# flybirdtian/pytorch_distributed_mnist

Measured on AMD Instinct MI355X. Metric: images/sec (whole node) MNIST CNN DDP at 1/2/4/8 MI355X, higher is better.
Workload: dtype bf16; 1 GPU; model=mnist_cnn, global_batch=256, batch_per_rank=256, parallelism=dp1, optimizer=sgd, graphs=True, grad_transport=local, epoch_steps=235, tail_batch_per_rank=96, conv2_products=bf16 MFMA, fp32 accumulation

## Files before the change

csrc/bind.cpp:

```cpp
#include <c10/core/DeviceGuard.h>
#include <c10/hip/HIPStream.h>
#include <torch/extension.h>

#include "kernels.h"
#include "xgmi.h"

namespace py = pybind11;

void xgmi_fill_exchange(py::handle reducer, int bucket, XgmiExch& x);
void register_comm(py::module& m);
void register_xgmi(py::module& m);

namespace {

hipStream_t cur_stream(const at::Tensor& t) {
  return c10::hip::getCurrentHIPStream(t.get_device()).stream();
}

void need(const at::Tensor& t, at::ScalarType dt, const char* name) {
  TORCH_CHECK(t.is_cuda(), name, " must be a HIP device tensor");
  TORCH_CHECK(t.scalar_type() == dt, name, " has dtype ", t.scalar_type(), ", expected ", dt);
  TORCH_CHECK(t.is_contiguous(), name, " must be contiguous");
}

void need_numel(const at::Tensor& t, int64_t n, const char* name) {
  TORCH_CHECK(t.numel() >= n, name, " has ", t.numel(), " elements, need >= ", n);
}

void need_aligned(const void* p, int bytes, const char* name) {
  TORCH_CHECK(reinterpret_cast<uintptr_t>(p) % bytes == 0, name, " must be ", bytes,
              "-byte aligned");
}

template <typename T>
T* ptr(const at::Tensor& t) { return reinterpret_cast<T*>(t.data_ptr()); }

unsigned* opt_sync(const c10::optional<at::Tensor>& t) {
  if (!t.has_value() || !t->defined()) return nullptr;
  TORCH_CHECK(t->is_cuda() && t->scalar_type() == at::kInt && t->is_contiguous() &&
                  t->numel() >= XG_LOC_WORDS, "xgmi sync words must be an int32 device tensor of ",
              XG_LOC_WORDS);
  return reinterpret_cast<unsigned*>(t->data_ptr());
}

unsigned* xg_step(const c10::optional<at::Tensor>& t) {
  unsigned* p = opt_sync(t);
  return p ? p + XG_LOC_STEP : nullptr;
}

int64_t* opt_i64(const c10::optional<at::Tensor>& t) {
  if (!t.has_value() || !t->defined()) return nullptr;
  need(*t, at::kLong, "counter");
  return ptr<int64_t>(*t);
}

LrSched opt_lr_sched(const c10::optional<py::tuple>& t, const int64_t* c1) {
  LrSched ls;
  if (!t.has_value()) return ls;
  TORCH_CHECK(t->size() == 3, "lr_sched: (table, cursor, lr)");
  TORCH_CHECK(c1 != nullptr, "lr_sched: the learning rate moves on with the optimizer-step "
                             "counter, which this launch does not advance (c1 is None)");
  const at::Tensor table = (*t)[0].cast<at::Tensor>();
  const at::Tensor cursor = (*t)[1].cast<at::Tensor>();
  const at::Tensor lr = (*t)[2].cast<at::Tensor>();
  need(table, at::kDouble, "lr_sched table");
  need(cursor, at::kLong, "lr_sched cursor");
  need(lr, at::kDouble, "lr_sched lr");
  TORCH_CHECK(table.numel() >= 1 && table.numel() <= INT32_MAX, "lr_sched table: 1..2^31-1 entries");
  TORCH_CHECK(cursor.numel() == 1 && lr.numel() == 1, "lr_sched cursor / lr: one element each");
  ls.table = table.data_ptr<double>();
  ls.n = (int)table.numel();
  ls.cursor = cursor.data_ptr<int64_t>();
  ls.lr = lr.data_ptr<double>();
  return ls;
}

float check_smoothing(double e) {
  TORCH_CHECK(e >= 0.0 && e <= 1.0, "label_smoothing must be in 0..1, got ", e);
  return (float)e;
}

void check_data(const at::Tensor& images, const at::Tensor& labels, const at::Tensor& idx,
                const at::Tensor& ctr, int64_t bfull, int64_t B) {
  need(images, at::kByte, "images");
  need(labels, at::kInt, "labels");
  need(idx, at::kInt, "idx");
  need(ctr, at::kLong, "ctr");
  TORCH_CHECK(images.dim() == 2 && images.size(1) == 784, "images must be [N, 784]");
  TORCH_CHECK(labels.numel() == images.size(0), "labels must be [N]");
  TORCH_CHECK(B >= 1 && B <= bfull, "batch ", B, " must be in [1, ", bfull, "]");
  TORCH_CHECK(ctr.numel() >= 1, "ctr must hold at least one counter");
  need_aligned(images.data_ptr(), 4, "images");
}

StepRows step_rows(int64_t bfull, int64_t spe, int64_t nrow) {
  if (spe > 0)
    TORCH_CHECK(nrow % 2 == 0 && (spe - 1) * bfull < nrow / 2 && spe * bfull >= nrow / 2,
                "epoch geometry: ", spe, " steps of ", bfull, " rows do not cover an epoch of ",
                nrow / 2, " rows");
  return StepRows{(int)bfull, (int)spe};
}

void lin_train(at::Tensor images, at::Tensor labels, c10::optional<at::Tensor> idx, at::Tensor ctr,
               int64_t bfull, int64_t B, at::Tensor W, at::Tensor b, at::Tensor slab,
               c10::optional<at::Tensor> metrics, c10::optional<at::Tensor> c1, int64_t spe,
               c10::optional<py::tuple> lr_sched, double label_smoothing) {
  c10::DeviceGuard g(images.device());
  const float eps = check_smoothing(label_smoothing);
  const bool gather = idx.has_value() && idx->defined();
  TORCH_CHECK(!(gather && spe > 0), "an epoch geometry needs the epoch buffer (idx None)");
  int64_t nrow;
  if (gather) {
    check_data(images, labels, *idx, ctr, bfull, B);
    nrow = idx->numel();
  } else {
    need(images, at::kByte, "images");
    need(labels, at::kInt, "labels");
    need(ctr, at::kLong, "ctr");
    TORCH_CHECK(images.dim() == 2 && images.size(1) == 784 && images.size(0) >= B,
                "images must be [>=B, 784]");
    TORCH_CHECK(labels.numel() == images.size(0), "labels must be [N]");
    TORCH_CHECK(B >= 1 && B <= bfull, "batch ", B, " must be in [1, ", bfull, "]");
    nrow = images.size(0);
  }
  need_aligned(images.data_ptr(), 16, "images");
  need(W, at::kFloat, "W");
  need(b, at::kFloat, "b");
  need(slab, at::kFloat, "slab");
  TORCH_CHECK(W.numel() == LIN_N * LIN_K && b.numel() == LIN_N, "W/b must be [10,784]/[10]");
  need_aligned(W.data_ptr(), 16, "W");
  const int64_t nblk = (B + LIN_ROWS - 1) / LIN_ROWS;
  need_numel(slab, nblk * LIN_SLAB, "slab");
  need_aligned(slab.data_ptr(), 16, "slab");
  double* mp = nullptr;
  if (metrics.has_value() && metrics->defined()) {
    need(*metrics, at::kDouble, "metrics");
    need_numel(*metrics, 3, "metrics");
    mp = metrics->data_ptr<double>();
  }
  launch_lin_train(images.data_ptr<uint8_t>(), labels.data_ptr<int32_t>(),
                   gather ? idx->data_ptr<int32_t>() : nullptr, nrow, ctr.data_ptr<int64_t>(),
                   step_rows(bfull, spe, nrow), (int)B, W.data_ptr<float>(), b.data_ptr<float>(),
                   slab.data_ptr<float>(), mp, opt_i64(c1), cur_stream(images),
                   opt_lr_sched(lr_sched, opt_i64(c1)), eps);
}

void lin_reduce(at::Tensor slab, int64_t B, at::Tensor gW, at::Tensor gb,
                c10::optional<at::Tensor> c0, c10::optional<at::Tensor> xg,
                c10::optional<at::Tensor> metrics) {
  c10::DeviceGuard g(slab.device());
  need(slab, at::kFloat, "slab");
  need(gW, at::kFloat, "gW");
  need(gb, at::kFloat, "gb");
  const int64_t nblk = (B + LIN_ROWS - 1) / LIN_ROWS;
  need_numel(slab, nblk * LIN_SLAB, "slab");
  TORCH_CHECK(gW.numel() == LIN_N * LIN_K && gb.numel() == LIN_N, "bad grad views");
  double* mp = nullptr;
  if (metrics.has_value() && metrics->defined()) {
    need(*metrics, at::kDouble, "metrics");
    need_numel(*metrics, 3, "metrics");
    mp = metrics->data_ptr<double>();
  }
  launch_lin_reduce(slab.data_ptr<float>(), (int)nblk, gW.data_ptr<float>(), gb.data_ptr<float>(),
                    opt_i64(c0), xg_step(xg), mp, cur_stream(slab));
}

void lin_eval(at::Tensor images, at::Tensor labels, at::Tensor W, at::Tensor b,
              at::Tensor metrics) {
  c10::DeviceGuard g(images.device());
  need(images, at::kByte, "images");
  need(labels, at::kInt, "labels");
  need(W, at::kFloat, "W");
  need(b, at::kFloat, "b");
  need(metrics, at::kDouble, "metrics");
  TORCH_CHECK(images.dim() == 2 && images.size(1) == 784, "images must be [N, 784]");
  TORCH_CHECK(labels.numel() == images.size(0), "labels must be [N]");
  TORCH_CHECK(W.numel() == LIN_N * LIN_K && b.numel() == LIN_N, "W/b must be [10,784]/[10]");
  need_numel(metrics, 3, "metrics");
  need_aligned(images.data_ptr(), 16, "images");
  need_aligned(W.data_ptr(), 16, "W");
  if (images.size(0) == 0) return;
  launch_lin_eval(images.data_ptr<uint8_t>(), labels.data_ptr<int32_t>(), (int)images.size(0),
                  W.data_ptr<float>(), b.data_ptr<float>(), metrics.data_ptr<double>(),
                  cur_stream(images));
}

void gather_epoch(at::Tensor images, at::Tensor labels, at::Tensor idx, at::Tensor out_images,
                  at::Tensor out_labels, c10::optional<at::Tensor> ctr, c10::optional<at::Tensor> step,
                  int64_t step_value, int64_t max_wgs) {
  c10::DeviceGuard g(images.device());
  need(images, at::kByte, "images");
  need(labels, at::kInt, "labels");
  need(out_images, at::kByte, "out_images");
  need(out_labels, at::kInt, "out_labels");
  TORCH_CHECK(idx.scalar_type() == at::kInt && idx.is_contiguous(), "idx must be contiguous int32");
  const int32_t* ip = nullptr;
  if (idx.is_cuda()) {
    ip = idx.data_ptr<int32_t>();
  } else {
    TORCH_CHECK(idx.is_pinned(), "a host idx must be pinned (device-mapped) memory");
    void* dp = nullptr;
    const hipError_t e = hipHostGetDevicePointer(&dp, idx.data_ptr(), 0);
    TORCH_CHECK(e == hipSuccess && dp != nullptr, "hipHostGetDevicePointer: ", hipGetErrorString(e));
    ip = static_cast<const int32_t*>(dp);
  }
  TORCH_CHECK(images.dim() == 2 && images.size(1) == 784, "images must be [N, 784]");
  const int64_t n = idx.numel();
  TORCH_CHECK(out_images.numel() >= n * 784 && out_labels.numel() >= n, "output too small");
  need_aligned(images.data_ptr(), 16, "images");
  need_aligned(out_images.data_ptr(), 16, "out_images");
  int64_t* cp = nullptr;
  int nctr = 0;
  if (ctr.has_value() && ctr->defined()) {
    need(*ctr, at::kLong, "ctr");
    TORCH_CHECK(ctr->numel() <= 256, "ctr: at most 256 counters");
    cp = ptr<int64_t>(*ctr);
    nctr = (int)ctr->numel();
  }
  int64_t* sp = nullptr;
  if (step.has_value() && step->defined()) {
    need(*step, at::kLong, "step");
    sp = ptr<int64_t>(*step);
  }
  launch_gather_epoch(images.data_ptr<uint8_t>(), labels.data_ptr<int32_t>(), ip, (int)n,
                      (int)images.size(0), out_images.data_ptr<uint8_t>(),
                      out_labels.data_ptr<int32_t>(), cp, nctr, sp, step_value, (int)max_wgs,
                      cur_stream(images));
}

void gather_epoch_augment(at::Tensor images, at::Tensor labels, at::Tensor idx,
                          at::Tensor out_images, at::Tensor out_labels,
                          c10::optional<at::Tensor> ctr, c10::optional<at::Tensor> step,
                          int64_t step_value, int64_t max_wgs, at::Tensor cosq, at::Tensor sinq,
                          at::Tensor invz, int64_t shift, int64_t epoch, uint64_t seed) {
  c10::DeviceGuard g(images.device());
  need(images, at::kByte, "images");
  need(labels, at::kInt, "labels");
  need(out_images, at::kByte, "out_images");
  need(out_labels, at::kInt, "out_labels");
  need(cosq, at::kInt, "cosq");
  need(sinq, at::kInt, "sinq");
  need(invz, at::kInt, "invz");
  need_numel(cosq, 1024, "cosq");
  need_numel(sinq, 1024, "sinq");
  need_numel(invz, 64, "invz");
  TORCH_CHECK(shift >= 0 && shift <= 8, "shift must be in 0..8, got ", shift);
  TORCH_CHECK(epoch >= 0 && epoch <= 0xffffffffLL, "epoch must fit 32 bits, got ", epoch);
  TORCH_CHECK(idx.scalar_type() == at::kInt && idx.is_contiguous(), "idx must be contiguous int32");
  const int32_t* ip = nullptr;
  if (idx.is_cuda()) {
    ip = idx.data_ptr<int32_t>();
  } else {
    TORCH_CHECK(idx.is_pinned(), "a host idx must be pinned (device-mapped) memory");
    void* dp = nullptr;
    const hipError_t e = hipHostGetDevicePointer(&dp, idx.data_ptr(), 0);
    TORCH_CHECK(e == hipSuccess && dp != nullptr, "hipHostGetDevicePointer: ", hipGetErrorString(e));
    ip = static_cast<const int32_t*>(dp);
  }
  TORCH_CHECK(images.dim() == 2 && images.size(1) == 784, "images must be [N, 784]");
  TORCH_CHECK(images.size(0) >= 1 && labels.numel() == images.size(0), "labels must be [N >= 1]");
  const int64_t n = idx.numel();
  TORCH_CHECK(out_images.numel() >= n * 784 && out_labels.numel() >= n, "output too small");
  need_aligned(images.data_ptr(), 16, "images");
  need_aligned(out_images.data_ptr(), 16, "out_images");
  int64_t* cp = nullptr;
  int nctr = 0;
  if (ctr.has_value() && ctr->defined()) {
    need(*ctr, at::kLong, "ctr");
    TORCH_CHECK(ctr->numel() <= 256, "ctr: at most 256 counters");
    cp = ptr<int64_t>(*ctr);
    nctr = (int)ctr->numel();
  }
  int64_t* sp = nullptr;
  if (step.has_value() && step->defined()) {
    need(*step, at::kLong, "step");
    sp = ptr<int64_t>(*step);
  }
  launch_gather_epoch_augment(images.data_ptr<uint8_t>(), labels.data_ptr<int32_t>(), ip, (int)n,
                              (int)images.size(0), out_images.data_ptr<uint8_t>(),
                              out_labels.data_ptr<int32_t>(), cp, nctr, sp, step_value,
                              (int)max_wgs, cosq.data_ptr<int32_t>(), sinq.data_ptr<int32_t>(),
                              invz.data_ptr<int32_t>(), (int)shift, (uint32_t)epoch, seed,
                              cur_stream(images));
}

void optim_step(int64_t kind, at::Tensor p, at::Tensor g, at::Tensor m, c10::optional<at::Tensor> v,
                at::Tensor lr, at::Tensor step, double beta1, double beta2, double eps, double wd,
                double momentum, double dampening, bool nesterov, double grad_scale,
                std::vector<py::tuple> segs, c10::optional<at::Tensor> xg, int64_t signal_ch,
                std::vector<int64_t> waits, double timeout_s, c10::optional<at::Tensor> bump,
                c10::optional<py::tuple> metrics, py::object xchg, int64_t xchg_bucket) {
  c10::DeviceGuard dg(p.device());
  need(p, at::kFloat, "params");
  need(g, at::kFloat, "grads");
  need(m, at::kFloat, "state m");
  need(lr, at::kDouble, "lr");
  need(step, at::kLong, "step");
  TORCH_CHECK(g.numel() == p.numel() && m.numel() == p.numel(), "arena size mismatch");
  TORCH_CHECK(kind == OPT_ADAM || kind == OPT_SGD, "bad optimizer kind");
  OptArgs a{};
  a.p = p.data_ptr<float>();
  a.g = g.data_ptr<float>();
  a.m = m.data_ptr<float>();
  a.v = nullptr;
  if (kind == OPT_ADAM) {
    TORCH_CHECK(v.has_value() && v->defined(), "adam needs exp_avg_sq");
    need(*v, at::kFloat, "state v");
    TORCH_CHECK(v->numel() == p.numel(), "arena size mismatch");
    a.v = v->data_ptr<float>();
  }
  a.lr = lr.data_ptr<double>();
  a.step = step.data_ptr<int64_t>();
  a.beta1_d = beta1;
  a.beta2_d = beta2;
  a.beta1 = (float)beta1;
  a.beta2 = (float)beta2;
  a.eps = (float)eps;
  a.wd = (float)wd;
  a.momentum = (float)momentum;
  a.dampening = (float)dampening;
  a.nesterov = nesterov ? 1 : 0;
  a.grad_scale = (float)grad_scale;
  TORCH_CHECK(!segs.empty() && segs.size() <= OPT_MAX_SEG, "1..8 optimizer segments");
  a.nseg = (int)segs.size();
  for (size_t i = 0; i < segs.size(); ++i) {
    const auto& t = segs[i];
    OptSeg& s = a.seg[i];
    s.offset = t[0].cast<int64_t>();
    s.rows = (int32_t)t[1].cast<int64_t>();
    s.cols = (int32_t)t[2].cast<int64_t>();
    TORCH_CHECK(s.offset >= 0 && s.rows >= 1 && s.cols >= 1 &&
                    s.offset + (int64_t)s.rows * s.cols <= p.numel(), "segment out of range");
    TORCH_CHECK(s.offset % 4 == 0, "segment offsets must be 16-byte aligned");
    s.shadow = nullptr;
    s.shadow_t = nullptr;
    s.shadow_lo = nullptr;
    s.slab = nullptr;
    s.nslab = 0;
    s.slab_col0 = 0;
    s.slab_stride = 0;
    s.wait_ch = -1;
    s.wait_mult = 0;
    if (!waits.empty()) {
      TORCH_CHECK(waits.size() == 2 * segs.size(), "waits must hold (channel, mult) per segment");
      s.wait_ch = (int32_t)waits[2 * i];
      s.wait_mult = (uint32_t)waits[2 * i + 1];
      TORCH_CHECK(s.wait_ch >= -1 && s.wait_ch < XG_MAX_CH, "bad wait channel");
    }
    if (t.size() > 5 && !t[5].is_none()) {
      auto sl = t[5].cast<py::tuple>();
      auto st = sl[0].cast<at::Tensor>();
      need(st, at::kFloat, "gradient slab");
      s.nslab = (int32_t)sl[1].cast<int64_t>();
      s.slab_col0 = (int32_t)sl[2].cast<int64_t>();
      s.slab_stride = sl[3].cast<int64_t>();
      const int64_t numel = (int64_t)s.rows * s.cols;
      TORCH_CHECK(s.nslab >= 1 && numel >= 4 && s.slab_col0 % 4 == 0 && s.slab_stride % 4 == 0 &&
                      s.slab_col0 + ((numel + 3) / 4) * 4 <= s.slab_stride &&
                      st.numel() >= (int64_t)s.nslab * s.slab_stride, "gradient slab geometry");
      need_aligned(st.data_ptr(), 16, "gradient slab");
      s.slab = st.data_ptr<float>();
    }
    if (!t[3].is_none()) {
      auto sh = t[3].cast<at::Tensor>();
      need(sh, at::kBFloat16, "shadow");
      TORCH_CHECK(sh.numel() == (int64_t)s.rows * s.cols, "shadow size mismatch");
      need_aligned(sh.data_ptr(), 8, "shadow");
      s.shadow = ptr<__bf16>(sh);
    }
    if (!t[4].is_none()) {
      auto sh = t[4].cast<at::Tensor>();
      need(sh, at::kBFloat16, "shadow_t");
      TORCH_CHECK(sh.numel() == (int64_t)s.rows * s.cols, "shadow_t size mismatch");
      s.shadow_t = ptr<__bf16>(sh);
    }
    if (t.size() > 9 && !t[9].is_none()) {
      auto sh = t[9].cast<at::Tensor>();
      need(sh, at::kBFloat16, "shadow_lo");
      TORCH_CHECK(sh.numel() == (int64_t)s.rows * s.cols, "shadow_lo size mismatch");
      need_aligned(sh.data_ptr(), 8, "shadow_lo");
      s.shadow_lo = ptr<__bf16>(sh);
    }
    s.tonly = (t.size() > 6 && !t[6].is_none() && t[6].cast<bool>()) ? 1 : 0;
    s.tfrag = (t.size() > 7 && !t[7].is_none() && t[7].cast<bool>()) ? 1 : 0;
    s.sfrag = (t.size() > 8 && !t[8].is_none() && t[8].cast<bool>()) ? 1 : 0;
    TORCH_CHECK(s.shadow_lo == nullptr || (s.shadow != nullptr && s.shadow_t == nullptr && !s.sfrag),
                "a lo shadow goes with a row-major shadow and no transposed copy");
    if (s.sfrag)
      TORCH_CHECK(s.shadow != nullptr && s.rows % 16 == 0 && s.cols % 32 == 0,
                  "a fragment-major shadow needs a 2-D segment with rows % 16 == 0 and cols % 32 == 0 "
                  "(a row shard of it starts on a 16-row fragment boundary)");
    if (s.tfrag)
      TORCH_CHECK(s.shadow_t != nullptr && s.rows % 32 == 0 && s.cols % 16 == 0,
                  "a fragment-major shadow_t needs rows % 32 == 0 and cols % 16 == 0");
    if (s.tonly) {
      TORCH_CHECK(s.shadow != nullptr && s.shadow_t != nullptr && s.slab == nullptr,
                  "a transpose-only segment needs shadow and shadow_t and no slab");
      need_aligned(s.shadow, 16, "shadow");
    }
  }
  a.xg = opt_sync(xg);
  a.xg_signal_ch = (int)signal_ch;
  a.xg_timeout = (long long)(timeout_s * 1e8);
  a.bump = opt_i64(bump);
  a.metrics = nullptr;
  a.mslab = nullptr;
  if (metrics.has_value()) {
    const auto& mt = *metrics;
    TORCH_CHECK(mt.size() == 5, "metrics: (slab, nslab, col, stride, metrics)");
    auto st = mt[0].cast<at::Tensor>();
    auto mv = mt[4].cast<at::Tensor>();
    need(st, at::kFloat, "metrics slab");
    need(mv, at::kDouble, "metrics");
    need_numel(mv, 3, "metrics");
    a.mnslab = (int32_t)mt[1].cast<int64_t>();
    a.mcol = (int32_t)mt[2].cast<int64_t>();
    a.mstride = mt[3].cast<int64_t>();
    TORCH_CHECK(a.mnslab >= 1 && a.mcol >= 0 && a.mcol + 2 <= a.mstride &&
                    st.numel() >= (int64_t)a.mnslab * a.mstride, "metrics slab geometry");
    a.mslab = st.data_ptr<float>();
    a.metrics = mv.data_ptr<double>();
  }
  TORCH_CHECK(signal_ch >= -1 && signal_ch < XG_MAX_CH, "bad signal channel");
  TORCH_CHECK(a.xg != nullptr || (signal_ch < 0 && waits.empty()),
              "optimizer waits / signals need the xgmi sync words");
  a.xx_on = 0;
  if (!xchg.is_none()) {
    xgmi_fill_exchange(xchg, (int)xchg_bucket, a.xx);
    a.xx_on = 1;
    int64_t blk = 0;
    bool plain_seen = false;
    for (int i = 0; i < a.nseg; ++i) {
      const OptSeg& sg = a.seg[i];
      if (sg.slab == nullptr) {
        plain_seen = true;
        continue;
      }
      TORCH_CHECK(!plain_seen, "exchange: slab segments must come first");
      TORCH_CHECK(sg.offset >= a.xx.off && sg.offset + (int64_t)sg.rows * sg.cols <= a.xx.off + a.xx.n,
                  "exchange: a slab segment outside the exchanged bucket");
      TORCH_CHECK(sg.wait_ch < 0, "exchange: slab segments wait for no channel");
      blk += ((int64_t)sg.rows * sg.cols + 63) / 64;
    }
    TORCH_CHECK(blk <= XG_XSLOTS, "exchange: ", blk, " slab workgroups exceed ", XG_XSLOTS, " slots");
  }
  launch_optim((int)kind, a, cur_stream(p));
}

void ema_update(at::Tensor params, at::Tensor ema, int64_t n, double w, bool warmup, double decay,
                at::Tensor step_word, int64_t offset, bool nt) {
  need(params, at::kFloat, "params");
  need(ema, at::kFloat, "ema");
  need(step_word, at::kLong, "step_word");
  c10::DeviceGuard g(params.device());
  TORCH_CHECK(ema.device() == params.device() && step_word.device() == params.device(),
              "params, ema and step_word must be on one device");
  TORCH_CHECK(n >= 1 && n <= params.numel() && n <= ema.numel(), "ema_update: n = ", n,
              " must be in 1..min(params, ema) = ", std::min(params.numel(), ema.numel()));
  TORCH_CHECK(step_word.numel() == 1, "step_word: one element");
  need_aligned(params.data_ptr(), 16, "params");
  need_aligned(ema.data_ptr(), 16, "ema");
  const char* pb = static_cast<const char*>(params.data_ptr());
  const char* eb = static_cast<const char*>(ema.data_ptr());
  TORCH_CHECK(pb + 4 * n <= eb || eb + 4 * n <= pb, "params and ema overlap");
  TORCH_CHECK(decay > 0.0 && decay < 1.0, "ema decay must be in (0, 1), got ", decay);
  TORCH_CHECK(w >= 0.0 && w <= 1.0 && (double)(float)w == w,
              "ema weight must be a float32 value in 0..1, got ", w);
  EmaArgs a;
  a.p = ptr<const float>(params);
  a.e = ptr<float>(ema);
  a.n = n;
  a.w = (float)w;
  a.warmup = warmup ? 1 : 0;
  a.decay = decay;
  a.step = ptr<const int64_t>(step_word);
  a.offset = offset;
  launch_ema_update(a, nt, cur_stream(params));
}

void xgmi_wait(at::Tensor sync, int64_t signal_ch, std::vector<int64_t> waits, double timeout_s) {
  c10::DeviceGuard g(sync.device());
  unsigned* loc = opt_sync(sync);
  TORCH_CHECK(waits.size() % 2 == 0 && waits.size() <= 8, "waits: up to 4 (channel, mult) pairs");
  TORCH_CHECK(signal_ch >= -1 && signal_ch < XG_MAX_CH, "bad signal channel");
  int ch[4];
  unsigned mult[4];
  const int n = (int)waits.size() / 2;
  for (int i = 0; i < n; ++i) {
    TORCH_CHECK(waits[2 * i] >= 0 && waits[2 * i] < XG_MAX_CH, "bad wait channel");
    ch[i] = (int)waits[2 * i];
    mult[i] = (unsigned)waits[2 * i + 1];
  }
  launch_xgmi_wait(loc, (int)signal_ch, n, ch, mult, (long long)(timeout_s * 1e8),
                   cur_stream(sync));
}

void debug_spin(double seconds) {
  TORCH_CHECK(seconds > 0 && seconds <= 30, "debug_spin: 0 < seconds <= 30");
  launch_debug_spin((long long)(seconds * 1e8), c10::hip::getCurrentHIPStream().stream());
}

void need_min(const at::Tensor& t, at::ScalarType dt, int64_t n, const char* name) {
  need(t, dt, name);
  need_numel(t, n, name);
  need_aligned(t.data_ptr(), 16, name);
}

static FcUpdate make_fc_update(const c10::optional<py::tuple>& t);

void cnn_fwd(at::Tensor images, at::Tensor labels, c10::optional<at::Tensor> idx,
             c10::optional<at::Tensor> ctr, int64_t bfull, int64_t B, at::Tensor w1, at::Tensor b1,
             at::Tensor w2, at::Tensor b2, at::Tensor pool, at::Tensor pmask,
             c10::optional<at::Tensor> xg, at::Tensor ylab, int64_t bands,
             c10::optional<at::Tensor> a1g, c10::optional<at::Tensor> xng, int64_t spe,
             c10::optional<py::tuple> fc_carry, c10::optional<py::tuple> fc_carry_wait) {
  c10::DeviceGuard g(images.device());
  FcUpdate fcc = make_fc_update(fc_carry);
  if (fc_carry_wait.has_value()) {
    const py::tuple& w = *fc_carry_wait;
    TORCH_CHECK(fcc.kind >= 0 && w.size() == 4, "fc_carry_wait: (sync, channel, mult, timeout_s) "
                "with fc_carry");
    fcc.wloc = opt_sync(w[0].cast<at::Tensor>());
    fcc.wch = (int)w[1].cast<int64_t>();
    fcc.wmult = (unsigned)w[2].cast<int64_t>();
    fcc.wtimeout = (long long)(w[3].cast<double>() * 1e8);
    TORCH_CHECK(fcc.wloc != nullptr && fcc.wch >= 0 && fcc.wch < XG_MAX_CH && fcc.wmult >= 1,
                "fc_carry_wait: bad channel / multiplier");
  }
  if (fcc.kind >= 0) {
    TORCH_CHECK(fcc.shadow_t_next != nullptr, "fc_carry: the W1^T copy (entry 16) is required");
    const bool training = (xg.has_value() && xg->defined()) || (a1g.has_value() && a1g->defined());
    TORCH_CHECK(training, "fc_carry: training launches only");
  }
  const FcUpdate* pfcc = fcc.kind >= 0 ? &fcc : nullptr;
  TORCH_CHECK(bands == 1 || bands == 2 || bands == 3 || bands == 6, "bands must be 1, 2, 3 or 6");
  const bool gather = idx.has_value() && idx->defined();
  const bool counted = ctr.has_value() && ctr->defined();
  if (gather) {
    TORCH_CHECK(counted, "ctr required with idx");
    check_data(images, labels, *idx, *ctr, bfull, B);
  } else if (counted) {
    need(images, at::kByte, "images");
    need(labels, at::kInt, "labels");
    need(*ctr, at::kLong, "ctr");
    TORCH_CHECK(images.dim() == 2 && images.size(1) == 784 && images.size(0) >= B, "images");
    TORCH_CHECK(B >= 1 && B <= bfull, "batch must be in [1, bfull]");
    need_aligned(images.data_ptr(), 4, "images");
  } else {
    need(images, at::kByte, "images");
    need(labels, at::kInt, "labels");
    TORCH_CHECK(images.dim() == 2 && images.size(1) == 784 && images.size(0) >= B,
                "images must be [>=B, 784]");
    need_aligned(images.data_ptr(), 4, "images");
  }
  TORCH_CHECK(B >= 1, "B must be >= 1");
  need(w1, at::kFloat, "w1");
  need(b1, at::kFloat, "b1");
  need(b2, at::kFloat, "b2");
  TORCH_CHECK(w1.numel() == 32 * 9 && b1.numel() == 32 && b2.numel() == 64, "conv1/conv2 bias");
  need_aligned(w1.data_ptr(), 16, "w1");
  need_aligned(b1.data_ptr(), 16, "b1");
  need_aligned(b2.data_ptr(), 16, "b2");
  need_min(w2, at::kBFloat16, 64 * 288, "w2");
  need_min(pool, at::kBFloat16, B * CNN_FEAT, "pool");
  need_min(pmask, at::kByte, B * CNN_FEAT, "pmask");
  need(ylab, at::kInt, "ylab");
  need_numel(ylab, B, "ylab");
  const bool train = xg.has_value() && xg->defined();
  if (train) need_min(*xg, at::kByte, B * 784, "xg");
  const int32_t* pidx = gather ? idx->data_ptr<int32_t>() : nullptr;
  const int64_t nrow = gather ? idx->numel() : images.size(0);
  const int64_t* pctr = counted ? ctr->data_ptr<int64_t>() : nullptr;
  uint8_t* pxg = train ? xg->data_ptr<uint8_t>() : nullptr;
  if (bands > 1) {
    __bf16* pa1 = nullptr;
    __bf16* pxn = nullptr;
    if (a1g.has_value() && a1g->defined()) {
      TORCH_CHECK(xng.has_value() && xng->defined(), "a1g needs xng");
      need_min(*a1g, at::kBFloat16, B * 676 * 32, "a1g");
      need_min(*xng, at::kBFloat16, B * 784, "xng");
      need_aligned(a1g->data_ptr(), 16, "a1g");
      need_aligned(xng->data_ptr(), 16, "xng");
      pa1 = ptr<__bf16>(*a1g);
      pxn = ptr<__bf16>(*xng);
    }
    launch_cnn_fwd_band(images.data_ptr<uint8_t>(), labels.data_ptr<int32_t>(), pidx, nrow, pctr,
                        step_rows(bfull, pidx ? 0 : spe, nrow), (int)B, (int)bands, w1.data_ptr<float>(), b1.data_ptr<float>(),
                        ptr<__bf16>(w2), b2.data_ptr<float>(), ptr<__bf16>(pool),
                        pmask.data_ptr<uint8_t>(), pa1, pxn, pxg, ylab.data_ptr<int32_t>(),
                        pfcc, cur_stream(images));
  } else {
    launch_cnn_fwd(images.data_ptr<uint8_t>(), labels.data_ptr<int32_t>(), pidx, nrow, pctr,
                   step_rows(bfull, pidx ? 0 : spe, nrow), (int)B, w1.data_ptr<float>(), b1.data_ptr<float>(), ptr<__bf16>(w2),
                   b2.data_ptr<float>(), ptr<__bf16>(pool), pmask.data_ptr<uint8_t>(), pxg,
                   ylab.data_ptr<int32_t>(), pfcc, cur_stream(images));
  }
}

void fc1_fwd(at::Tensor pool, at::Tensor wf1, at::Tensor part, int64_t B, int64_t splitk) {
  c10::DeviceGuard g(pool.device());
  TORCH_CHECK(B >= 1, "B must be >= 1");
  TORCH_CHECK(splitk >= 1 && (32 % splitk == 0 || 96 % splitk == 0),
              "splitk must divide 32 or 96");
  need_min(pool, at::kBFloat16, B * CNN_FEAT, "pool");
  need_min(wf1, at::kBFloat16, (int64_t)CNN_HID * CNN_FEAT, "wf1");
  need_min(part, at::kFloat, splitk * B * CNN_HID, "part");
  launch_fc1_fwd(ptr<__bf16>(pool), ptr<__bf16>(wf1), part.data_ptr<float>(), (int)B, (int)splitk,
                 cur_stream(pool));
}

struct HeadOut {
  __bf16 *dh = nullptr, *dht = nullptr;
  float *slab = nullptr, *dh32 = nullptr;
};

HeadOut check_head(const at::Tensor& part, int64_t splitk, int64_t B, const at::Tensor& bf1,
                   const at::Tensor& wf2, const at::Tensor& bf2, const at::Tensor& ylab, bool train,
                   const c10::optional<at::Tensor>& dh, const c10::optional<at::Tensor>& dht,
                   int64_t ldt, const c10::optional<at::Tensor>& slab, const at::Tensor& metrics,
                   const c10::optional<at::Tensor>& dh32) {
  TORCH_CHECK(B >= 1, "B must be >= 1");
  need_min(part, at::kFloat, splitk * B * CNN_HID, "part");
  need_min(bf1, at::kFloat, CNN_HID, "bf1");
  need_min(wf2, at::kFloat, CNN_NCLS * CNN_HID, "wf2");
  need(bf2, at::kFloat, "bf2");
  TORCH_CHECK(bf2.numel() == CNN_NCLS, "bf2");
  need(ylab, at::kInt, "ylab");
  need_numel(ylab, B, "ylab");
  need(metrics, at::kDouble, "metrics");
  need_numel(metrics, 3, "metrics");
  HeadOut o;
  if (train) {
    TORCH_CHECK(ldt % 32 == 0 && ldt >= B, "ldt must be a multiple of 32 and >= B");
    TORCH_CHECK(slab, "train mode needs slab");
    if (dh32.has_value() && dh32->defined()) {
      need_min(*dh32, at::kFloat, ldt * CNN_HID, "dh32");
      need_aligned(dh32->data_ptr(), 8, "dh32");
      o.dh32 = dh32->data_ptr<float>();
    } else {
      TORCH_CHECK(dh && dht, "train mode needs dh and dht (or dh32)");
      need_min(*dh, at::kBFloat16, ldt * CNN_HID, "dh");
      need_min(*dht, at::kBFloat16, ldt * CNN_HID, "dht");
      o.dh = ptr<__bf16>(*dh);
      o.dht = ptr<__bf16>(*dht);
    }
    need_min(*slab, at::kFloat, (int64_t)cnn_head_blocks((int)(ldt / CNN_HEAD_ROWS)) * CNN_HEAD_SLAB,
             "head slab");
    o.slab = slab->data_ptr<float>();
  }
  return o;
}

void cnn_head(at::Tensor part, int64_t splitk, int64_t B, at::Tensor bf1, at::Tensor wf2,
              at::Tensor bf2, at::Tensor ylab, bool train, c10::optional<at::Tensor> dh,
              c10::optional<at::Tensor> dht, int64_t ldt, c10::optional<at::Tensor> slab,
              at::Tensor metrics, c10::optional<at::Tensor> c0, c10::optional<at::Tensor> c1,
              c10::optional<at::Tensor> xg, c10::optional<at::Tensor> dh32,
              c10::optional<py::tuple> lr_sched) {
  c10::DeviceGuard g(part.device());
  TORCH_CHECK(train || !lr_sched.has_value(), "lr_sched: only a training head advances it");
  const HeadOut o = check_head(part, splitk, B, bf1, wf2, bf2, ylab, train, dh, dht, ldt, slab,
                               metrics, dh32);
  launch_cnn_head(part.data_ptr<float>(), (int)splitk, (int)B, bf1.data_ptr<float>(),
                  wf2.data_ptr<float>(), bf2.data_ptr<float>(), ylab.data_ptr<int32_t>(), train, o.dh,
                  o.dht, (int)ldt, o.slab, metrics.data_ptr<double>(), opt_i64(c0), opt_i64(c1),
                  train ? xg_step(xg) : nullptr, o.dh32, cur_stream(part),
                  opt_lr_sched(lr_sched, opt_i64(c1)));
}

void cnn_head_smooth(at::Tensor part, int64_t splitk, int64_t B, at::Tensor bf1, at::Tensor wf2,
                     at::Tensor bf2, at::Tensor ylab, c10::optional<at::Tensor> dh,
                     c10::optional<at::Tensor> dht, int64_t ldt, c10::optional<at::Tensor> slab,
                     at::Tensor metrics, c10::optional<at::Tensor> c0, c10::optional<at::Tensor> c1,
                     c10::optional<at::Tensor> xg, c10::optional<at::Tensor> dh32,
                     double label_smoothing, c10::optional<py::tuple> lr_sched) {
  c10::DeviceGuard g(part.device());
  const HeadOut o = check_head(part, splitk, B, bf1, wf2, bf2, ylab, true, dh, dht, ldt, slab,
                               metrics, dh32);
  const float eps = check_smoothing(label_smoothing);
  launch_cnn_head_smooth(part.data_ptr<float>(), (int)splitk, (int)B, bf1.data_ptr<float>(),
                         wf2.data_ptr<float>(), bf2.data_ptr<float>(), ylab.data_ptr<int32_t>(),
                         o.dh, o.dht, (int)ldt, o.slab, opt_i64(c0), opt_i64(c1), xg_step(xg),
                         o.dh32, eps, cur_stream(part), opt_lr_sched(lr_sched, opt_i64(c1)));
}

const uint32_t* check_dropout(const at::Tensor& epoch, int64_t T) {
  need(epoch, at::kInt, "epoch");
  need_numel(epoch, 1, "epoch");
  TORCH_CHECK(T >= 0 && T <= (int64_t)DROPOUT_MAX_T, "T must be in 0..", DROPOUT_MAX_T, ", got ", T);
  return reinterpret_cast<const uint32_t*>(epoch.data_ptr<int32_t>());
}

void cnn_head_dropout(at::Tensor part, int64_t splitk, int64_t B, at::Tensor bf1, at::Tensor wf2,
                      at::Tensor bf2, at::Tensor ylab, c10::optional<at::Tensor> dh,
                      c10::optional<at::Tensor> dht, int64_t ldt, c10::optional<at::Tensor> slab,
                      at::Tensor metrics, c10::optional<at::Tensor> c0,
                      c10::optional<at::Tensor> c1, c10::optional<at::Tensor> xg,
                      c10::optional<at::Tensor> dh32, at::Tensor epoch, uint64_t seed, int64_t T,
                      double scale, c10::optional<py::tuple> lr_sched, double label_smoothing) {
  c10::DeviceGuard g(part.device());
  const HeadOut o = check_head(part, splitk, B, bf1, wf2, bf2, ylab, true, dh, dht, ldt, slab,
                               metrics, dh32);
  const uint32_t* pe = check_dropout(epoch, T);
  TORCH_CHECK(scale >= 1.0 && scale <= 65536.0 / (65536.0 - DROPOUT_MAX_T) + 1e-6,
              "scale must be 65536 / (65536 - T), got ", scale);
  const float eps = check_smoothing(label_smoothing);
  launch_cnn_head_dropout(part.data_ptr<float>(), (int)splitk, (int)B, bf1.data_ptr<float>(),
                          wf2.data_ptr<float>(), bf2.data_ptr<float>(), ylab.data_ptr<int32_t>(),
                          o.dh, o.dht, (int)ldt, o.slab, opt_i64(c0), opt_i64(c1), xg_step(xg),
                          o.dh32, pe, seed, (uint32_t)T, (float)scale, cur_stream(part),
                          opt_lr_sched(lr_sched, opt_i64(c1)), eps);
}

at::Tensor dropout_mask_rows(at::Tensor ylab, at::Tensor epoch, uint64_t seed, int64_t T) {
  c10::DeviceGuard g(ylab.device());
  need(ylab, at::kInt, "ylab");
  TORCH_CHECK(ylab.dim() == 1 && ylab.numel() >= 1, "ylab must be [B >= 1]");
  const uint32_t* pe = check_dropout(epoch, T);
  const int64_t B = ylab.numel();
  at::Tensor out = at::empty({B, (int64_t)CNN_HID}, ylab.options().dtype(at::kByte));
  launch_dropout_mask_rows(ylab.data_ptr<int32_t>(), (int)B, pe, seed, (uint32_t)T,
                           out.data_ptr<uint8_t>(), cur_stream(ylab));
  return out;
}

struct PredictOut {
  float* logp;
  int32_t* pred;
  int64_t* confusion;
  double* metrics;
};
PredictOut check_predict_out(int64_t B, bool labelled, const at::Tensor& logp, const at::Tensor& pred,
                             const c10::optional<at::Tensor>& confusion,
                             const c10::optional<at::Tensor>& metrics) {
  PredictOut o{};
  need(logp, at::kFloat, "logp");
  need_numel(logp, B * CNN_NCLS, "logp");
  need(pred, at::kInt, "pred");
  need_numel(pred, B, "pred");
  o.logp = logp.data_ptr<float>();
  o.pred = pred.data_ptr<int32_t>();
  if (confusion.has_value() && confusion->defined()) {
    TORCH_CHECK(labelled, "confusion needs labels");
    need(*confusion, at::kLong, "confusion");
    TORCH_CHECK(confusion->numel() == CNN_NCLS * CNN_NCLS, "confusion must be [10, 10]");
    o.confusion = confusion->data_ptr<int64_t>();
  }
  if (metrics.has_value() && metrics->defined()) {
    TORCH_CHECK(labelled, "metrics need labels");
    need(*metrics, at::kDouble, "metrics");
    need_numel(*metrics, 3, "metrics");
    o.metrics = metrics->data_ptr<double>();
  }
  return o;
}

void cnn_predict_head(at::Tensor part, int64_t splitk, int64_t B, at::Tensor bf1, at::Tensor wf2,
                      at::Tensor bf2, c10::optional<at::Tensor> ylab, at::Tensor logp,
                      at::Tensor pred, c10::optional<at::Tensor> confusion,
                      c10::optional<at::Tensor> metrics) {
  c10::DeviceGuard g(part.device());
  TORCH_CHECK(B >= 1 && B <= INT32_MAX / (CNN_NCLS * 4), "B must be in [1, 2^31 / 40)");
  TORCH_CHECK(splitk >= 1, "splitk must be >= 1");
  need_min(part, at::kFloat, splitk * B * CNN_HID, "part");
  need_min(bf1, at::kFloat, CNN_HID, "bf1");
  need_min(wf2, at::kFloat, CNN_NCLS * CNN_HID, "wf2");
  need(bf2, at::kFloat, "bf2");
  TORCH_CHECK(bf2.numel() == CNN_NCLS, "bf2");
  const bool labelled = ylab.has_value() && ylab->defined();
  if (labelled) {
    need(*ylab, at::kInt, "ylab");
    need_numel(*ylab, B, "ylab");
  }
  const PredictOut o = check_predict_out(B, labelled, logp, pred, confusion, metrics);
  launch_cnn_predict_head(part.data_ptr<float>(), (int)splitk, (int)B, bf1.data_ptr<float>(),
                          wf2.data_ptr<float>(), bf2.data_ptr<float>(),
                          labelled ? ylab->data_ptr<int32_t>() : nullptr, o.logp, o.pred,
                          o.confusion, o.metrics, cur_stream(part));
}

void lin_predict(at::Tensor images, c10::optional<at::Tensor> labels, at::Tensor W, at::Tensor b,
                 at::Tensor logp, at::Tensor pred, c10::optional<at::Tensor> confusion,
                 c10::optional<at::Tensor> metrics) {
  c10::DeviceGuard g(images.device());
  need(images, at::kByte, "images");
  need(W, at::kFloat, "W");
  need(b, at::kFloat, "b");
  TORCH_CHECK(images.dim() == 2 && images.size(1) == 784, "images must be [N, 784]");
  const int64_t n = images.size(0);
  TORCH_CHECK(n <= INT32_MAX / LIN_K, "too many rows for one launch");
  const bool labelled = labels.has_value() && labels->defined();
  if (labelled) {
    need(*labels, at::kInt, "labels");
    TORCH_CHECK(labels->numel() == n, "labels must be [N]");
  }
  TORCH_CHECK(W.numel() == LIN_N * LIN_K && b.numel() == LIN_N, "W/b must be [10,784]/[10]");
  need_aligned(images.data_ptr(), 16, "images");
  need_aligned(W.data_ptr(), 16, "W");
  const PredictOut o = check_predict_out(n, labelled, logp, pred, confusion, metrics);
  if (n == 0) return;
  launch_lin_predict(images.data_ptr<uint8_t>(), labelled ? labels->data_ptr<int32_t>() : nullptr,
                     (int)n, W.data_ptr<float>(), b.data_ptr<float>(), o.logp, o.pred, o.confusion,
                     o.metrics, cur_stream(images));
}


static FcUpdate make_fc_update(const c10::optional<py::tuple>& t) {
  FcUpdate u{};
  u.kind = -1;
  if (!t.has_value()) return u;
  const py::tuple& a = *t;
  TORCH_CHECK(a.size() >= 16 && a.size() <= 18, "fc_update: 16 to 18 entries");
  u.kind = (int)a[0].cast<int64_t>();
  TORCH_CHECK(u.kind == OPT_SGD, "fc_update: SGD-momentum only (Adam runs in the optimizer kernel)");
  auto p = a[1].cast<at::Tensor>(), g = a[2].cast<at::Tensor>(), m = a[3].cast<at::Tensor>();
  auto sh = a[5].cast<at::Tensor>(), lr = a[6].cast<at::Tensor>(), st = a[7].cast<at::Tensor>();
  need(p, at::kFloat, "fc p");
  need(g, at::kFloat, "fc g");
  need(m, at::kFloat, "fc m");
  need(sh, at::kBFloat16, "fc shadow");
  need(lr, at::kDouble, "lr");
  need(st, at::kLong, "step");
  u.numel = p.numel();
  TORCH_CHECK(u.numel == (int64_t)CNN_HID * CNN_FEAT && g.numel() == u.numel &&
                  m.numel() == u.numel && sh.numel() == u.numel, "fc_update: fc1 weight sizes");
  for (const void* q : {p.data_ptr(), g.data_ptr(), m.data_ptr()}) need_aligned(q, 16, "fc_update fp32");
  need_aligned(sh.data_ptr(), 16, "fc_update shadow");
  u.p = p.data_ptr<float>();
  u.g = g.data_ptr<float>();
  u.m = m.data_ptr<float>();
  u.v = nullptr;
  u.shadow = ptr<__bf16>(sh);
  u.lr = lr.data_ptr<double>();
  u.step = st.data_ptr<int64_t>();
  u.beta1_d = a[8].cast<double>();
  u.beta2_d = a[9].cast<double>();
  u.beta1 = (float)u.beta1_d;
  u.beta2 = (float)u.beta2_d;
  u.eps = (float)a[10].cast<double>();
  u.wd = (float)a[11].cast<double>();
  u.momentum = (float)a[12].cast<double>();
  u.dampening = (float)a[13].cast<double>();
  u.nesterov = a[14].cast<bool>() ? 1 : 0;
  u.grad_scale = (float)a[15].cast<double>();
  u.shadow_t_next = nullptr;
  u.store_grad = (a.size() == 18 && !a[17].is_none()) ? (a[17].cast<bool>() ? 1 : 0) : 1;
  if (a.size() >= 17 && !a[16].is_none()) {
    auto t2 = a[16].cast<at::Tensor>();
    need(t2, at::kBFloat16, "fc shadow_t_next");
    TORCH_CHECK(t2.numel() == u.numel, "fc_update: shadow_t_next is one W1^T copy");
    need_aligned(t2.data_ptr(), 16, "fc_update shadow_t_next");
    u.shadow_t_next = ptr<__bf16>(t2);
  }
  return u;
}

void fc1_bwd(at::Tensor dh, at::Tensor dht, int64_t ldt, at::Tensor pool, at::Tensor wf1t,
             int64_t B, at::Tensor gwf1, at::Tensor dpool, at::Tensor head_slab, at::Tensor gwf2,
             at::Tensor gbf2, at::Tensor gbf1, at::Tensor metrics,
             c10::optional<py::tuple> fc_update) {
  c10::DeviceGuard g(dh.device());
  TORCH_CHECK(B >= 1 && ldt % 32 == 0 && ldt >= B, "bad ldt/B");
  need_min(dh, at::kBFloat16, ldt * CNN_HID, "dh");
  need_min(dht, at::kBFloat16, ldt * CNN_HID, "dht");
  need_min(pool, at::kBFloat16, B * CNN_FEAT, "pool");
  need_min(wf1t, at::kBFloat16, (int64_t)CNN_FEAT * CNN_HID, "wf1t");
  need_min(dpool, at::kBFloat16, B * CNN_FEAT, "dpool");
  need(gwf1, at::kFloat, "gwf1");
  need(gwf2, at::kFloat, "gwf2");
  need(gbf2, at::kFloat, "gbf2");
  need(gbf1, at::kFloat, "gbf1");
  TORCH_CHECK(gwf1.numel() == (int64_t)CNN_HID * CNN_FEAT && gwf2.numel() == CNN_NCLS * CNN_HID &&
                  gbf2.numel() == CNN_NCLS && gbf1.numel() == CNN_HID, "fc grad views");
  const int64_t hb = cnn_head_blocks((int)(ldt / CNN_HEAD_ROWS));
  need_min(head_slab, at::kFloat, hb * CNN_HEAD_SLAB, "head slab");
  need(metrics, at::kDouble, "metrics");
  need_numel(metrics, 3, "metrics");
  const FcUpdate fcu = make_fc_update(fc_update);
  if (fcu.shadow_t_next != nullptr) {
    const char* r0 = reinterpret_cast<const char*>(wf1t.data_ptr());
    const char* w0 = reinterpret_cast<const char*>(fcu.shadow_t_next);
    const int64_t nb = (int64_t)CNN_FEAT * CNN_HID * 2;
    TORCH_CHECK(w0 + nb <= r0 || r0 + nb <= w0, "fc_update: shadow_t_next overlaps the W1^T being read");
  }
  launch_fc1_bwd(ptr<__bf16>(dh), ptr<__bf16>(dht), (int)ldt, ptr<__bf16>(pool), ptr<__bf16>(wf1t),
                 (int)B, gwf1.data_ptr<float>(), ptr<__bf16>(dpool), head_slab.data_ptr<float>(),
                 (int)hb, gwf2.data_ptr<float>(), gbf2.data_ptr<float>(), gbf1.data_ptr<float>(),
                 metrics.data_ptr<double>(), fcu, cur_stream(dh));
}

static int64_t conv_blocks(int64_t B, int64_t ipb, int64_t bands) {
  return bands > 1 ? B * bands : (int64_t)cnn_bwd_blocks((int)B, (int)ipb);
}

void cnn_bwd(at::Tensor xg, at::Tensor w1, at::Tensor b1, at::Tensor dpool, at::Tensor pmask,
             at::Tensor w2t, int64_t B, int64_t ipb, at::Tensor slab,
             c10::optional<at::Tensor> xg_sync, int64_t bands, c10::optional<at::Tensor> a1g,
             c10::optional<at::Tensor> xng) {
  c10::DeviceGuard g(xg.device());
  TORCH_CHECK(B >= 1 && ipb >= 1, "bad B/ipb");
  TORCH_CHECK(bands == 1 || ((bands == 2 || bands == 3 || bands == 6) && ipb == 1),
              "bands must be 1, or 2 / 3 / 6 with one image per band group");
  need_min(xg, at::kByte, B * 784, "xg");
  need(w1, at::kFloat, "w1");
  need(b1, at::kFloat, "b1");
  TORCH_CHECK(w1.numel() == 32 * 9 && b1.numel() == 32, "conv1 weight/bias");
  need_min(dpool, at::kBFloat16, B * CNN_FEAT, "dpool");
  need_min(pmask, at::kByte, B * CNN_FEAT, "pmask");
  need_min(w2t, at::kBFloat16, 288 * 64, "w2t");
  need_min(slab, at::kFloat, conv_blocks(B, ipb, bands) * CNN_CONV_SLAB, "conv slab");
  need_aligned(slab.data_ptr(), 16, "conv slab");
  if (bands > 1) {
    TORCH_CHECK(a1g.has_value() && xng.has_value(), "the band backward needs a1g and xng");
    need_min(*a1g, at::kBFloat16, B * 676 * 32, "a1g");
    need_min(*xng, at::kBFloat16, B * 784, "xng");
    need_aligned(a1g->data_ptr(), 16, "a1g");
    need_aligned(xng->data_ptr(), 16, "xng");
    launch_cnn_bwd_band(ptr<__bf16>(*a1g), ptr<__bf16>(*xng), ptr<__bf16>(dpool),
                        pmask.data_ptr<uint8_t>(), ptr<__bf16>(w2t), (int)B, (int)bands,
                        slab.data_ptr<float>(), opt_sync(xg_sync), cur_stream(xg));
  } else
    launch_cnn_bwd(xg.data_ptr<uint8_t>(), w1.data_ptr<float>(), b1.data_ptr<float>(),
                   ptr<__bf16>(dpool), pmask.data_ptr<uint8_t>(), ptr<__bf16>(w2t), (int)B, (int)ipb,
                   slab.data_ptr<float>(), opt_sync(xg_sync), cur_stream(xg));
}

void conv_reduce(at::Tensor slab, int64_t nblk, at::Tensor gw2, at::Tensor gb2, at::Tensor gw1,
                 at::Tensor gb1) {
  c10::DeviceGuard g(slab.device());
  need_min(slab, at::kFloat, nblk * CNN_CONV_SLAB, "conv slab");
  need_aligned(slab.data_ptr(), 16, "conv slab");
  TORCH_CHECK(nblk >= 1, "nblk must be >= 1");
  need(gw2, at::kFloat, "gw2");
  need(gb2, at::kFloat, "gb2");
  need(gw1, at::kFloat, "gw1");
  need(gb1, at::kFloat, "gb1");
  TORCH_CHECK(gw2.numel() == 64 * 288 && gb2.numel() == 64 && gw1.numel() == 288 &&
                  gb1.numel() == 32, "conv grad views");
  launch_conv_reduce(slab.data_ptr<float>(), (int)nblk, gw2.data_ptr<float>(),
                     gb2.data_ptr<float>(), gw1.data_ptr<float>(), gb1.data_ptr<float>(),
                     cur_stream(slab));
}

int64_t cnn_bwd_nblk(int64_t B, int64_t ipb, int64_t bands) { return conv_blocks(B, ipb, bands); }

static float* w2x_ptr(const c10::optional<at::Tensor>& w2x) {
  TORCH_CHECK(w2x.has_value() && w2x->defined(), "the split-bf16 path needs the w2x buffer");
  need_min(*w2x, at::kFloat, 2 * 9 * 32 * 128 / 4, "w2x");
  need_aligned(w2x->data_ptr(), 16, "w2x");
  return w2x->data_ptr<float>();
}

void f32_fwd(at::Tensor images, at::Tensor labels, c10::optional<at::Tensor> ctr, int64_t bfull,
             int64_t B, at::Tensor w1, at::Tensor b1, at::Tensor w2, at::Tensor b2,
             at::Tensor pool, c10::optional<at::Tensor> pmask, c10::optional<at::Tensor> a1g,
             c10::optional<at::Tensor> xng, at::Tensor ylab, int64_t spe, bool x3,
             c10::optional<at::Tensor> w2x, c10::optional<at::Tensor> w2s) {
  c10::DeviceGuard g(images.device());
  need(images, at::kByte, "images");
  need(labels, at::kInt, "labels");
  TORCH_CHECK(images.dim() == 2 && images.size(1) == 784 && images.size(0) >= 1, "images [N, 784]");
  TORCH_CHECK(labels.numel() == images.size(0), "labels [N]");
  need_aligned(images.data_ptr(), 4, "images");
  TORCH_CHECK(B >= 1 && (!ctr.has_value() ? images.size(0) >= B : B <= bfull), "batch size");
  if (ctr.has_value()) need(*ctr, at::kLong, "ctr");
  need(w1, at::kFloat, "w1");
  need(b1, at::kFloat, "b1");
  need(w2, at::kFloat, "w2");
  need(b2, at::kFloat, "b2");
  TORCH_CHECK(w1.numel() == 288 && b1.numel() == 32 && w2.numel() == 64 * 288 && b2.numel() == 64,
              "conv weights");
  for (const void* q : {w1.data_ptr(), b1.data_ptr(), b2.data_ptr()}) need_aligned(q, 16, "conv weight");
  need_min(pool, at::kFloat, B * CNN_FEAT, "pool");
  need(ylab, at::kInt, "ylab");
  need_min(ylab, at::kInt, B, "ylab");
  const __bf16* w2sp = nullptr;
  if (x3) {
    TORCH_CHECK(w2s.has_value() && w2s->defined(), "the split-bf16 forward needs w2s");
    need(*w2s, at::kBFloat16, "w2s");
    TORCH_CHECK(w2s->numel() == 2 * 64 * 288, "w2s: hi / lo planes of conv2's weight");
    need_aligned(w2s->data_ptr(), 16, "w2s");
    w2sp = ptr<__bf16>(*w2s);
  }
  const bool train = a1g.has_value() && a1g->defined();
  if (train) {
    TORCH_CHECK(pmask.has_value() && xng.has_value(), "training needs pmask, a1g and xng");
    need_min(*pmask, at::kByte, B * CNN_FEAT, "pmask");
    need_min(*a1g, at::kFloat, B * 676 * 32, "a1g");
    need_min(*xng, at::kFloat, B * 784, "xng");
    need_aligned(a1g->data_ptr(), 16, "a1g");
    need_aligned(xng->data_ptr(), 16, "xng");
  }
  launch_f32_fwd(images.data_ptr<uint8_t>(), labels.data_ptr<int32_t>(), images.size(0),
                 ctr.has_value() ? ctr->data_ptr<int64_t>() : nullptr,
                 step_rows(bfull, ctr.has_value() ? spe : 0, images.size(0)), (int)B,
                 w1.data_ptr<float>(), b1.data_ptr<float>(), w2.data_ptr<float>(), b2.data_ptr<float>(),
                 pool.data_ptr<float>(), train ? pmask->data_ptr<uint8_t>() : nullptr,
                 train ? a1g->data_ptr<float>() : nullptr, train ? xng->data_ptr<float>() : nullptr,
                 ylab.data_ptr<int32_t>(), x3,
                 train && x3 ? w2x_ptr(w2x) : nullptr, w2sp, cur_stream(images));
}

void f32_fc1_fwd(at::Tensor pool, at::Tensor w1, at::Tensor part, int64_t B, int64_t splitk,
                 bool x3) {
  c10::DeviceGuard g(pool.device());
  TORCH_CHECK(B >= 1 && splitk >= 1 && 288 % splitk == 0, "splitk must divide 288");
  TORCH_CHECK(!x3 || 96 % splitk == 0, "split-bf16 fc1: splitk must divide 96");
  need_min(pool, at::kFloat, B * CNN_FEAT, "pool");
  need(w1, at::kFloat, "w1");
  TORCH_CHECK(w1.numel() == (int64_t)CNN_HID * CNN_FEAT, "fc1 weight");
  need_min(part, at::kFloat, splitk * B * CNN_HID, "part");
  for (const void* q : {pool.data_ptr(), w1.data_ptr()}) need_aligned(q, 16, "fc1 operand");
  launch_f32_fc1_fwd(pool.data_ptr<float>(), w1.data_ptr<float>(), part.data_ptr<float>(), (int)B,
                     (int)splitk, x3, cur_stream(pool));
}

void f32_fc1_bwd(at::Tensor dh, int64_t ldt, at::Tensor pool, at::Tensor w1, int64_t B,
                 at::Tensor gwf1, at::Tensor dpool, at::Tensor head_slab, at::Tensor gwf2,
                 at::Tensor gbf2, at::Tensor gbf1, at::Tensor metrics, bool x3) {
  c10::DeviceGuard g(dh.device());
  TORCH_CHECK(B >= 1 && ldt % 32 == 0 && ldt >= B, "ldt must be a multiple of 32 and >= B");
  need_min(dh, at::kFloat, ldt * CNN_HID, "dh32");
  need_min(pool, at::kFloat, B * CNN_FEAT, "pool");
  need(w1, at::kFloat, "w1");
  TORCH_CHECK(w1.numel() == (int64_t)CNN_HID * CNN_FEAT, "fc1 weight");
  need(gwf1, at::kFloat, "gwf1");
  TORCH_CHECK(gwf1.numel() == (int64_t)CNN_HID * CNN_FEAT, "fc1 grad");
  need_min(dpool, at::kFloat, B * CNN_FEAT, "dpool");
  const int hb = cnn_head_blocks((int)(ldt / CNN_HEAD_ROWS));
  need_min(head_slab, at::kFloat, (int64_t)hb * CNN_HEAD_SLAB, "head slab");
  need(gwf2, at::kFloat, "gwf2");
  need(gbf2, at::kFloat, "gbf2");
  need(gbf1, at::kFloat, "gbf1");
  TORCH_CHECK(gwf2.numel() == 1280 && gbf2.numel() == 10 && gbf1.numel() == 128, "head grads");
  need(metrics, at::kDouble, "metrics");
  need_numel(metrics, 3, "metrics");
  for (const void* q : {dh.data_ptr(), pool.data_ptr(), w1.data_ptr()}) need_aligned(q, 16, "fc1 operand");
  launch_f32_fc1_bwd(dh.data_ptr<float>(), (int)ldt, pool.data_ptr<float>(), w1.data_ptr<float>(),
                     (int)B, gwf1.data_ptr<float>(), dpool.data_ptr<float>(),
                     head_slab.data_ptr<float>(), hb, gwf2.data_ptr<float>(), gbf2.data_ptr<float>(),
                     gbf1.data_ptr<float>(), metrics.data_ptr<double>(), x3, cur_stream(dh));
}

void f32_conv_bwd(at::Tensor a1g, at::Tensor xng, at::Tensor dpool, at::Tensor pmask, at::Tensor w2,
                  int64_t B, at::Tensor slab, int64_t ipb, bool x3, c10::optional<at::Tensor> w2x) {
  c10::DeviceGuard g(a1g.device());
  TORCH_CHECK(B >= 1 && ipb >= 1, "B and ipb must be >= 1");
  need_min(a1g, at::kFloat, B * 676 * 32, "a1g");
  need_min(xng, at::kFloat, B * 784, "xng");
  need_min(dpool, at::kFloat, B * CNN_FEAT, "dpool");
  need_min(pmask, at::kByte, B * CNN_FEAT, "pmask");
  need(w2, at::kFloat, "w2");
  TORCH_CHECK(w2.numel() == 64 * 288, "conv2 weight");
  need_min(slab, at::kFloat, (int64_t)f32_conv_bwd_blocks((int)B, (int)ipb, x3) * CNN_CONV_SLAB,
           "conv slab");
  launch_f32_conv_bwd(a1g.data_ptr<float>(), xng.data_ptr<float>(), dpool.data_ptr<float>(),
                      pmask.data_ptr<uint8_t>(), w2.data_ptr<float>(), (int)B, (int)ipb,
                      slab.data_ptr<float>(), x3, x3 ? w2x_ptr(w2x) : nullptr, cur_stream(a1g));
}

void graph_upload(int64_t exec, int64_t device) {
  TORCH_CHECK(exec != 0, "graph_upload: graph is not instantiated");
  c10::DeviceGuard g(c10::Device(c10::kCUDA, (c10::DeviceIndex)device));
  hipStream_t s = c10::hip::getCurrentHIPStream((c10::DeviceIndex)device).stream();
  hipError_t e = hipGraphUpload(reinterpret_cast<hipGraphExec_t>(exec), s);
  TORCH_CHECK(e == hipSuccess, "hipGraphUpload: ", hipGetErrorString(e));
}

at::Tensor read_stamps(const std::string& which) {
  at::Tensor t = at::zeros({256, 16}, at::TensorOptions().dtype(at::kLong));
  auto* p = reinterpret_cast<unsigned long long*>(t.data_ptr<int64_t>());
  if (which == "fwd") read_stamps_fwd(p);
  else if (which == "head") read_stamps_head(p);
  else if (which == "fc1_bwd") read_stamps_fc1_bwd(p);
  else if (which == "fwd_band") read_stamps_fwd_band(p);
  else if (which == "bwd_band") read_stamps_bwd_band(p);
  else if (which == "f32") read_stamps_f32(p);
  else read_stamps_bwd(p);
  return t;
}

}

PYBIND11_MODULE(_C, m) {
  m.doc() = "MI355X (gfx950) kernels + RCCL runtime for pytorch_distributed_mnist_amd";
#ifdef PDM_DEBUG_BOUNDS
  m.attr("DEBUG_BOUNDS") = true;
#else
  m.attr("DEBUG_BOUNDS") = false;
#endif
  m.attr("LIN_ROWS") = LIN_ROWS;
  m.attr("LIN_SLAB") = LIN_SLAB;
  m.attr("OPT_ADAM") = OPT_ADAM;
  m.attr("OPT_SGD") = OPT_SGD;
  m.attr("XG_LOC_ERR") = XG_LOC_ERR;
  m.attr("XG_LOC_STEP") = XG_LOC_STEP;
  m.attr("XG_LOC_READY") = XG_LOC_READY;
  m.attr("XG_LOC_DONE") = XG_LOC_DONE;
  m.def("lin_train", &lin_train, py::arg("images"), py::arg("labels"), py::arg("idx"),
        py::arg("ctr"), py::arg("bfull"), py::arg("B"), py::arg("W"), py::arg("b"), py::arg("slab"),
        py::arg("metrics") = py::none(), py::arg("c1") = py::none(), py::arg("spe") = 0,
        py::arg("lr_sched") = py::none(), py::arg("label_smoothing") = 0.0);
  m.def("lin_reduce", &lin_reduce, py::arg("slab"), py::arg("B"), py::arg("gW"), py::arg("gb"),
        py::arg("c0") = py::none(), py::arg("xg") = py::none(), py::arg("metrics") = py::none());
  m.def("lin_eval", &lin_eval);
  m.def("optim_step", &optim_step, py::arg("kind"), py::arg("p"), py::arg("g"), py::arg("m"),
        py::arg("v"), py::arg("lr"), py::arg("step"), py::arg("beta1"), py::arg("beta2"),
        py::arg("eps"), py::arg("wd"), py::arg("momentum"), py::arg("dampening"),
        py::arg("nesterov"), py::arg("grad_scale"), py::arg("segs"), py::arg("xg") = py::none(),
        py::arg("signal_ch") = -1, py::arg("waits") = std::vector<int64_t>{},
        py::arg("timeout_s") = 60.0, py::arg("bump") = py::none(),
        py::arg("metrics") = py::none(), py::arg("xchg") = py::none(), py::arg("xchg_bucket") = 1);
  m.def("ema_update", &ema_update, py::arg("params"), py::arg("ema"), py::arg("n"), py::arg("w"),
        py::arg("warmup"), py::arg("decay"), py::arg("step_word"), py::arg("offset"),
        py::arg("nt") = false);
  m.def("gather_epoch", &gather_epoch, py::arg("images"), py::arg("labels"), py::arg("idx"),
        py::arg("out_images"), py::arg("out_labels"), py::arg("ctr") = py::none(),
        py::arg("step") = py::none(), py::arg("step_value") = 0, py::arg("max_wgs") = 0);
  m.def("gather_epoch_augment", &gather_epoch_augment, py::arg("images"), py::arg("labels"),
        py::arg("idx"), py::arg("out_images"), py::arg("out_labels"), py::arg("ctr") = py::none(),
        py::arg("step") = py::none(), py::arg("step_value") = 0, py::arg("max_wgs") = 0,
        py::arg("cosq"), py::arg("sinq"), py::arg("invz"), py::arg("shift"), py::arg("epoch"),
        py::arg("seed"));
  m.def("xgmi_wait", &xgmi_wait);
  m.def("debug_spin", &debug_spin, py::arg("seconds"));
  m.attr("CNN_HEAD_ROWS") = CNN_HEAD_ROWS;
  m.def("cnn_head_nblk", [](int64_t ldt) { return cnn_head_blocks((int)(ldt / CNN_HEAD_ROWS)); });
  m.attr("CNN_HEAD_SLAB") = CNN_HEAD_SLAB;
  m.attr("CNN_CONV_SLAB") = CNN_CONV_SLAB;
  m.attr("CNN_CONV_SLAB_DB2") = CNN_CONV_SLAB_DB2;
  m.attr("CNN_CONV_SLAB_DW1") = CNN_CONV_SLAB_DW1;
  m.attr("CNN_CONV_SLAB_DB1") = CNN_CONV_SLAB_DB1;
  m.def("cnn_fwd", &cnn_fwd, py::arg("images"), py::arg("labels"), py::arg("idx"), py::arg("ctr"),
        py::arg("bfull"), py::arg("B"), py::arg("w1"), py::arg("b1"), py::arg("w2"), py::arg("b2"),
        py::arg("pool"), py::arg("pmask"), py::arg("xg"), py::arg("ylab"), py::arg("bands") = 1,
        py::arg("a1g") = py::none(), py::arg("xng") = py::none(), py::arg("spe") = 0,
        py::arg("fc_carry") = py::none(), py::arg("fc_carry_wait") = py::none());
  m.def("fc1_fwd", &fc1_fwd);
  m.attr("FC1_BIG_B") = FC1_BIG_B;
  m.def("cnn_head", &cnn_head, py::arg("part"), py::arg("splitk"), py::arg("B"), py::arg("bf1"),
        py::arg("wf2"), py::arg("bf2"), py::arg("ylab"), py::arg("train"), py::arg("dh"),
        py::arg("dht"), py::arg("ldt"), py::arg("slab"), py::arg("metrics"), py::arg("c0"),
        py::arg("c1"), py::arg("xg") = py::none(), py::arg("dh32") = py::none(),
        py::arg("lr_sched") = py::none());
  m.def("cnn_head_dropout", &cnn_head_dropout, py::arg("part"), py::arg("splitk"), py::arg("B"),
        py::arg("bf1"), py::arg("wf2"), py::arg("bf2"), py::arg("ylab"), py::arg("dh"),
        py::arg("dht"), py::arg("ldt"), py::arg("slab"), py::arg("metrics"), py::arg("c0"),
        py::arg("c1"), py::arg("xg") = py::none(), py::arg("dh32") = py::none(), py::arg("epoch"),
        py::arg("seed"), py::arg("T"), py::arg("scale"), py::arg("lr_sched") = py::none(),
        py::arg("label_smoothing") = 0.0);
  m.def("cnn_head_smooth", &cnn_head_smooth, py::arg("part"), py::arg("splitk"), py::arg("B"),
        py::arg("bf1"), py::arg("wf2"), py::arg("bf2"), py::arg("ylab"), py::arg("dh"),
        py::arg("dht"), py::arg("ldt"), py::arg("slab"), py::arg("metrics"), py::arg("c0"),
        py::arg("c1"), py::arg("xg") = py::none(), py::arg("dh32") = py::none(),
        py::arg("label_smoothing"), py::arg("lr_sched") = py::none());
  m.def("dropout_mask_rows", &dropout_mask_rows, py::arg("ylab"), py::arg("epoch"),
        py::arg("seed"), py::arg("T"));
  m.def("cnn_predict_head", &cnn_predict_head, py::arg("part"), py::arg("splitk"), py::arg("B"),
        py::arg("bf1"), py::arg("wf2"), py::arg("bf2"), py::arg("ylab"), py::arg("logp"),
        py::arg("pred"), py::arg("confusion") = py::none(), py::arg("metrics") = py::none());
  m.def("lin_predict", &lin_predict, py::arg("images"), py::arg("labels"), py::arg("W"),
        py::arg("b"), py::arg("logp"), py::arg("pred"), py::arg("confusion") = py::none(),
        py::arg("metrics") = py::none());
  m.def("fc1_bwd", &fc1_bwd, py::arg("dh"), py::arg("dht"), py::arg("ldt"), py::arg("pool"),
        py::arg("wf1t"), py::arg("B"), py::arg("gwf1"), py::arg("dpool"), py::arg("head_slab"),
        py::arg("gwf2"), py::arg("gbf2"), py::arg("gbf1"), py::arg("metrics"),
        py::arg("fc_update") = py::none());
  m.def("cnn_bwd", &cnn_bwd, py::arg("xg"), py::arg("w1"), py::arg("b1"), py::arg("dpool"),
        py::arg("pmask"), py::arg("w2t"), py::arg("B"), py::arg("ipb"), py::arg("slab"),
        py::arg("xg_sync") = py::none(), py::arg("bands") = 1, py::arg("a1g") = py::none(),
        py::arg("xng") = py::none());
  m.def("conv_reduce", &conv_reduce);
  m.def("f32_fwd", &f32_fwd, py::arg("images"), py::arg("labels"), py::arg("ctr"), py::arg("bfull"),
        py::arg("B"), py::arg("w1"), py::arg("b1"), py::arg("w2"), py::arg("b2"), py::arg("pool"),
        py::arg("pmask"), py::arg("a1g"), py::arg("xng"), py::arg("ylab"), py::arg("spe") = 0,
        py::arg("x3") = false, py::arg("w2x") = py::none(), py::arg("w2s") = py::none());
  m.def("f32_fc1_fwd", &f32_fc1_fwd, py::arg("pool"), py::arg("w1"), py::arg("part"), py::arg("B"),
        py::arg("splitk"), py::arg("x3") = false);
  m.def("f32_fc1_bwd", &f32_fc1_bwd, py::arg("dh"), py::arg("ldt"), py::arg("pool"), py::arg("w1"),
        py::arg("B"), py::arg("gwf1"), py::arg("dpool"), py::arg("head_slab"), py::arg("gwf2"),
        py::arg("gbf2"), py::arg("gbf1"), py::arg("metrics"), py::arg("x3") = false);
  m.def("f32_conv_bwd", &f32_conv_bwd, py::arg("a1g"), py::arg("xng"), py::arg("dpool"),
        py::arg("pmask"), py::arg("w2"), py::arg("B"), py::arg("slab"), py::arg("ipb") = 1,
        py::arg("x3") = false, py::arg("w2x") = py::none());
  m.def("f32_conv_bwd_nblk", [](int64_t B, int64_t ipb, bool x3) {
    return (int64_t)f32_conv_bwd_blocks((int)B, (int)ipb, x3); }, py::arg("B"), py::arg("ipb") = 1,
    py::arg("x3") = false);
  m.def("cnn_bwd_nblk", &cnn_bwd_nblk, py::arg("B"), py::arg("ipb"), py::arg("bands") = 1);
  m.def("read_stamps", &read_stamps);
  m.def("graph_upload", &graph_upload);
  register_comm(m);
  register_xgmi(m);
}
```

csrc/kernels.h:

```cpp
#pragma once
#include <hip/hip_runtime.h>
#include <stdint.h>

#include "xgmi.h"


struct StepRows {
  int bfull;
  int spe;
};
__host__ __device__ __forceinline__ int64_t step_row(const StepRows g, int64_t nrow, int64_t c,
                                                     int img) {
  if (g.spe <= 0) return c * g.bfull + img;
  const uint32_t e = (uint32_t)c / (uint32_t)g.spe;
  const int64_t s = c - (int64_t)e * g.spe;
  return (int64_t)(e & 1u) * (nrow >> 1) + s * g.bfull + img;
}

struct LrSched {
  const double* table = nullptr;
  int n = 0;
  int64_t* cursor = nullptr;
  double* lr = nullptr;
};

constexpr int LIN_K = 784;
constexpr int LIN_N = 10;
constexpr int LIN_ROWS = 4;
constexpr int LIN_SLAB = 7856;
constexpr int LIN_EVAL_ROWS = 16;

void launch_lin_train(const uint8_t* images, const int32_t* labels, const int32_t* idx,
                      int64_t nrow, const int64_t* ctr, StepRows sr, int B, const float* W, const float* b,
                      float* slab, double* metrics, int64_t* c1, hipStream_t st,
                      LrSched ls = LrSched(), float label_smoothing = 0.f);
void launch_lin_reduce(const float* slab, int nblk, float* gW, float* gb, int64_t* c0, unsigned* c2,
                       double* metrics, hipStream_t st);
void launch_lin_eval(const uint8_t* images, const int32_t* labels, int n_total, const float* W,
                     const float* b, double* metrics, hipStream_t st);

void launch_gather_epoch(const uint8_t* images, const int32_t* labels, const int32_t* idx, int n,
                         int nimg, uint8_t* out_images, int32_t* out_labels, int64_t* ctr,
                         int nctr, int64_t* step, int64_t step_value, int max_wgs, hipStream_t st);
void launch_gather_epoch_augment(const uint8_t* images, const int32_t* labels, const int32_t* idx,
                                 int n, int nimg, uint8_t* out_images, int32_t* out_labels,
                                 int64_t* ctr, int nctr, int64_t* step, int64_t step_value,
                                 int max_wgs, const int32_t* cosq, const int32_t* sinq,
                                 const int32_t* invz, int shift, uint32_t epoch, uint64_t seed,
                                 hipStream_t st);

constexpr int OPT_ADAM = 0;
constexpr int OPT_SGD = 1;
constexpr int OPT_MAX_SEG = 8;

struct OptSeg {
  int64_t offset;
  int32_t rows, cols;
  int32_t first_block;
  __bf16* shadow;
  __bf16* shadow_t;
  __bf16* shadow_lo;
  const float* slab;
  int32_t nslab, slab_col0;
  int64_t slab_stride;
  int32_t wait_ch;
  uint32_t wait_mult;
  int32_t tonly;
  int32_t tfrag;
  int32_t sfrag;
};

__host__ __device__ inline int64_t frag_pos(int64_t m, int64_t k, int32_t K) {
  return (((m >> 4) * (K >> 5) + (k >> 5)) * 64 + ((k >> 3) & 3) * 16 + (m & 15)) * 8 + (k & 7);
}
__host__ __device__ inline int64_t shadow_pos(int32_t sfrag, int32_t cols, int64_t row, int64_t col) {
  return sfrag ? frag_pos(row, col, cols) : row * cols + col;
}
__host__ __device__ inline int64_t shadow_t_pos(int32_t tfrag, int32_t rows, int64_t row, int64_t col) {
  return tfrag ? frag_pos(col, row, rows) : col * rows + row;
}

struct OptArgs {
  float* p;
  const float* g;
  float* m;
  float* v;
  const double* lr;
  const int64_t* step;
  double beta1_d, beta2_d;
  float beta1, beta2, eps, wd, momentum, dampening;
  int nesterov;
  float grad_scale;
  int nseg;
  OptSeg seg[OPT_MAX_SEG];
  unsigned* xg;
  int xg_signal_ch;
  long long xg_timeout;
  int64_t* bump;
  const float* mslab;
  int32_t mnslab, mcol;
  int64_t mstride;
  double* metrics;
  int xx_on;
  XgmiExch xx;
};

void launch_optim(int kind, OptArgs& a, hipStream_t st);

struct EmaArgs {
  const float* p;
  float* e;
  int64_t n;
  float w;
  int warmup;
  double decay;
  const int64_t* step;
  int64_t offset;
};
void launch_ema_update(const EmaArgs& a, bool nt, hipStream_t st);

constexpr int FC1_BIG_B = 2048;

struct FcUpdate {
  int kind;
  int64_t numel;
  float* p;
  const float* g;
  float* m;
  float* v;
  __bf16* shadow;
  __bf16* shadow_t_next;
  const double* lr;
  const int64_t* step;
  double beta1_d, beta2_d;
  float beta1, beta2, eps, wd, momentum, dampening;
  int nesterov;
  float grad_scale;
  int store_grad;
  unsigned* wloc;
  int wch;
  unsigned wmult;
  long long wtimeout;
};

constexpr int CNN_FEAT = 9216;
constexpr int CNN_HID = 128;
constexpr int CNN_NCLS = 10;
constexpr int CNN_HEAD_ROWS = 4;
constexpr int CNN_HEAD_MAX_BLOCKS = 256;
int cnn_head_blocks(int groups);
constexpr int CNN_HEAD_SLAB = 1420;
constexpr int CNN_CONV_SLAB = 18816;
constexpr int CNN_CONV_SLAB_DB2 = 18432;
constexpr int CNN_CONV_SLAB_DW1 = 18496;
constexpr int CNN_CONV_SLAB_DB1 = 18784;

void launch_cnn_fwd(const uint8_t* images, const int32_t* labels, const int32_t* idx,
                    int64_t nrow, const int64_t* ctr, StepRows sr, int B, const float* w1, const float* b1,
                    const __bf16* w2, const float* b2, __bf16* pool, uint8_t* pmask, uint8_t* xg,
                    int32_t* ylab, const FcUpdate* fcc, hipStream_t st);
void launch_cnn_fwd_band(const uint8_t* images, const int32_t* labels, const int32_t* idx,
                         int64_t nrow, const int64_t* ctr, StepRows sr, int B, int bands,
                         const float* w1, const float* b1, const __bf16* w2, const float* b2,
                         __bf16* pool, uint8_t* pmask, __bf16* a1g, __bf16* xng, uint8_t* xg,
                         int32_t* ylab, const FcUpdate* fcc, hipStream_t st);
void launch_fc1_fwd(const __bf16* pool, const __bf16* wf1, float* part, int B, int splitk,
                    hipStream_t st);
void launch_cnn_head(const float* part, int splitk, int B, const float* bf1, const float* wf2,
                     const float* bf2, const int32_t* ylab, bool train, __bf16* dh, __bf16* dht,
                     int ldt, float* slab, double* metrics, int64_t* c0, int64_t* c1,
                     unsigned* c2, float* dh32, hipStream_t st, LrSched ls = LrSched());
void launch_cnn_head_smooth(const float* part, int splitk, int B, const float* bf1,
                            const float* wf2, const float* bf2, const int32_t* ylab, __bf16* dh,
                            __bf16* dht, int ldt, float* slab, int64_t* c0, int64_t* c1,
                            unsigned* c2, float* dh32, float label_smoothing, hipStream_t st,
                            LrSched ls = LrSched());
void launch_cnn_head_dropout(const float* part, int splitk, int B, const float* bf1,
                             const float* wf2, const float* bf2, const int32_t* ylab, __bf16* dh,
                             __bf16* dht, int ldt, float* slab, int64_t* c0, int64_t* c1,
                             unsigned* c2, float* dh32, const uint32_t* epoch, uint64_t seed,
                             uint32_t T, float scale, hipStream_t st, LrSched ls = LrSched(),
                             float label_smoothing = 0.f);
void launch_dropout_mask_rows(const int32_t* ylab, int B, const uint32_t* epoch, uint64_t seed,
                              uint32_t T, uint8_t* out, hipStream_t st);
constexpr uint32_t DROPOUT_MAX_T = 58982;
void launch_fc1_bwd(const __bf16* dh, const __bf16* dht, int ldt, const __bf16* pool,
                    const __bf16* wf1t, int B, float* gwf1, __bf16* dpool, const float* head_slab,
                    int head_blocks, float* gwf2, float* gbf2, float* gbf1, double* metrics,
                    const FcUpdate& fcu, hipStream_t st);
void launch_cnn_bwd(const uint8_t* xg, const float* w1, const float* b1, const __bf16* dpool,
                    const uint8_t* pmask, const __bf16* w2t, int B, int imgs_per_block, float* slab,
                    unsigned* xg_sync, hipStream_t st);
int cnn_bwd_blocks(int B, int imgs_per_block);
void launch_cnn_bwd_band(const __bf16* a1g, const __bf16* xng, const __bf16* dpool,
                         const uint8_t* pmask, const __bf16* w2t, int B, int bands, float* slab,
                         unsigned* xg_sync, hipStream_t st);
void launch_conv_reduce(const float* slab, int nblk, float* gw2, float* gb2, float* gw1, float* gb1,
                        hipStream_t st);

void launch_f32_fwd(const uint8_t* images, const int32_t* labels, int64_t nrow, const int64_t* ctr,
                    StepRows sr, int B, const float* w1, const float* b1, const float* w2,
                    const float* b2, float* pool, uint8_t* pmask, float* a1g, float* xng,
                    int32_t* ylab, bool x3, float* w2x, const __bf16* w2s, hipStream_t st);
void launch_f32_fc1_fwd(const float* pool, const float* w1, float* part, int B, int splitk,
                        bool x3, hipStream_t st);
void launch_f32_fc1_bwd(const float* dh, int ldt, const float* pool, const float* w1, int B,
                        float* gwf1, float* dpool, const float* head_slab, int head_blocks,
                        float* gwf2, float* gbf2, float* gbf1, double* metrics, bool x3, hipStream_t st);
int f32_conv_bwd_blocks(int B, int per, bool x3);
void launch_f32_conv_bwd(const float* a1g, const float* xng, const float* dpool,
                         const uint8_t* pmask, const float* w2, int B, int ipb, float* slab,
                         bool x3, const float* w2x, hipStream_t st);

void launch_cnn_predict_head(const float* part, int splitk, int B, const float* bf1,
                             const float* wf2, const float* bf2, const int32_t* ylab, float* logp,
                             int32_t* pred, int64_t* confusion, double* metrics, hipStream_t st);
void launch_lin_predict(const uint8_t* images, const int32_t* labels, int n_total, const float* W,
                        const float* b, float* logp, int32_t* pred, int64_t* confusion,
                        double* metrics, hipStream_t st);

void read_stamps_fwd(unsigned long long* host);
void read_stamps_head(unsigned long long* host);
void read_stamps_fc1_bwd(unsigned long long* host);
void read_stamps_bwd(unsigned long long* host);
void read_stamps_fwd_band(unsigned long long* host);
void read_stamps_bwd_band(unsigned long long* host);
void read_stamps_f32(unsigned long long* host);
```

csrc/kernels/cnn_fwd.hip:

```cpp
#include "cnn_common.h"
#include "fc_carry.h"

namespace {

using namespace cnn;

constexpr int FWD_THREADS = 512;
constexpr int F_X3 = 0;
constexpr int F_A1 = 6400;
constexpr int F_PS = F_A1 + P1 * 64;
constexpr int F_MS = F_PS + PP * C2 * 2;
constexpr int F_LUT = F_MS + PP * C2;
constexpr int F_W = F_LUT + 512;
constexpr int F_TOTAL = F_W + 1536;
static_assert(2 * F_TOTAL <= 163840 && F_A1 % 128 == 0, "cnn_fwd LDS carve");

template <bool TRAIN, bool CARRY>
__global__ __launch_bounds__(FWD_THREADS, 2) void cnn_fwd_kernel(
    const uint8_t* __restrict__ images, const int32_t* __restrict__ labels,
    const int32_t* __restrict__ idx, int64_t nrow, const int64_t* __restrict__ ctr, const StepRows sr,
    const float* __restrict__ w1, const float* __restrict__ b1, const bf16* __restrict__ w2,
    const float* __restrict__ b2, bf16* __restrict__ pool, uint8_t* __restrict__ pmask,
    uint8_t* __restrict__ xg, int32_t* __restrict__ ylab, const FcUpdate fcc, int nconv) {
  __shared__ __attribute__((aligned(16))) char smem[F_TOTAL];
  static_assert(F_TOTAL >= FCC_LDS + 4, "carried fc1 update tiles fit the forward's LDS");
  if constexpr (CARRY) {
    if ((int)blockIdx.x >= nconv) {
      fc_carry_role(fcc, blockIdx.x - nconv, gridDim.x - nconv, smem);
      return;
    }
  }
  bf16x4* x3 = reinterpret_cast<bf16x4*>(smem + F_X3);
  char* a1s = smem + F_A1;
  bf16* ps = reinterpret_cast<bf16*>(smem + F_PS);
  uint8_t* ms = reinterpret_cast<uint8_t*>(smem + F_MS);

  const int img = blockIdx.x;
  const int tid = threadIdx.x, lane = tid & 63;
  const int wave = __builtin_amdgcn_readfirstlane(tid >> 6);
  const int g = lane >> 4, i16 = lane & 15;
  PDM_STAMP(0);
  float4 wq = make_float4(0.f, 0.f, 0.f, 0.f);
  const int wt = tid - 256;
  if (wt >= 0 && wt < 96) {
    const float4* srcw = wt < 72 ? reinterpret_cast<const float4*>(w1) + wt
                         : wt < 80 ? reinterpret_cast<const float4*>(b1) + (wt - 72)
                                   : reinterpret_cast<const float4*>(b2) + (wt - 80);
    wq = *srcw;
  }
  __builtin_amdgcn_sched_barrier(0);
  const int64_t row_u = ctr ? step_row(sr, nrow, *ctr, img) : (int64_t)img;
  PDM_CHECK(row_u < nrow, "cnn_fwd sample row past the epoch", row_u, nrow);
  const int64_t row = min(row_u, nrow - 1);
  const int64_t src = idx ? (int64_t)idx[row] : row;
  uint32_t xw = 0, xn = 0;
  if (tid < 196) {
    xw = reinterpret_cast<const uint32_t*>(images + src * 784)[tid];
    xn = reinterpret_cast<const uint32_t*>(images + src * 784)[min(tid + 1, 195)];
  }
  int lab = 0;
  if (tid == 64) {
    int vz;
    asm volatile("v_mov_b32 %0, 0" : "=v"(vz));
    lab = labels[src + vz];
  }
  if (tid == 0) PDM_STAMP_VAL(8, PDM_CLOCK());
  bf16* lut = reinterpret_cast<bf16*>(smem + F_LUT);
  if (tid >= 256) lut[tid - 256] = to_bf16(pdm_normalize(tid - 256));
  float* wl = reinterpret_cast<float*>(smem + F_W);
  if (wt >= 0 && wt < 96) reinterpret_cast<float4*>(wl)[wt] = wq;
  __builtin_amdgcn_sched_barrier(0);
  __syncthreads();

  float w1v[2][4];
#pragma unroll
  for (int j = 0; j < 4; ++j)
#pragma unroll
    for (int mt = 0; mt < 2; ++mt)
      w1v[mt][j] = wl[(mt * 16 + i16) * 9 + 3 * min(g, 2) + min(j, 2)];
  f32x4 b1v[2];
#pragma unroll
  for (int mt = 0; mt < 2; ++mt) b1v[mt] = reinterpret_cast<const f32x4*>(wl + 288)[mt * 4 + g];
  if (tid < 196) {
    const bf16 v[6] = {lut[xw & 0xff], lut[(xw >> 8) & 0xff], lut[(xw >> 16) & 0xff],
                       lut[xw >> 24], lut[xn & 0xff], lut[(xn >> 8) & 0xff]};
#pragma unroll
    for (int i = 0; i < 4; ++i) x3[4 * tid + i] = bf16x4{v[i], v[i + 1], v[i + 2], bf16{}};
    if (TRAIN) st_ho<4>(reinterpret_cast<uint32_t*>(xg + (int64_t)img * 784) + tid, xw);
    if (tid == 0) PDM_STAMP_VAL(9, PDM_CLOCK());
  }
  __syncthreads();
  PDM_STAMP(1);

  __builtin_amdgcn_sched_barrier(0);
  const int nh = wave & 1;
  float b2r[2];
#pragma unroll
  for (int j = 0; j < 2; ++j) b2r[j] = wl[320 + nh * 32 + j * 16 + i16];
  bf16x8 wb[9][2];
  auto load_wb = [&](int f) {
#pragma unroll
    for (int e = 3 * f; e < 3 * f + 3; ++e)
      wb[e >> 1][e & 1] = *reinterpret_cast<const bf16x8*>(
          w2 + ((int64_t)((nh * 2 + (e & 1)) * 9 + (e >> 1)) * 64 + lane) * 8);
  };

  bf16x4 w1f[2];
#pragma unroll
  for (int mt = 0; mt < 2; ++mt)
#pragma unroll
    for (int j = 0; j < 4; ++j) w1f[mt][j] = to_bf16(g < 3 && j < 3 ? w1v[mt][j] : 0.f);
  {
    constexpr int TPW = 6;
    const int rowg = IMG * (g < 3 ? g : 0);
    const int a1c = (conv1_pair_chunk(g) ^ (i16 & 3)) << 4;
#pragma unroll
    for (int h = 0; h < TPW; h += 3) {
    bf16x4 bx[TPW];
    int vv[TPW];
#pragma unroll
    for (int k = h; k < h + 3; ++k) {
      vv[k] = (wave + 8 * k) * 16 + i16;
      bx[k] = x3[min(vv[k], IMG * H1 - 1) + rowg];
    }
#pragma unroll
    for (int k = h; k < h + 3; ++k) {
      load_wb(k);
      const int y = vv[k] / IMG, x = vv[k] - y * IMG;
      const bool ok = y < H1 && x < H1;
      bf16x4 o[2];
#pragma unroll
      for (int mt = 0; mt < 2; ++mt) {
        f32x4 acc = __builtin_amdgcn_mfma_f32_16x16x16bf16_1k(w1f[mt], bx[k], b1v[mt], 0, 0, 0);
        o[mt] = bf16x4{to_bf16(relu1(acc[0])), to_bf16(relu1(acc[1])),
                       to_bf16(relu1(acc[2])), to_bf16(relu1(acc[3]))};
      }
      const int dst = ok ? F_A1 + (vv[k] - 2 * y) * 64 + a1c : F_PS + lane * 16;
      *reinterpret_cast<uint4*>(smem + dst) = conv1_pair(o[0], o[1]);
    }
    }
  }
  __syncthreads();
  PDM_STAMP(2);

  const int q = i16 >> 2, s = i16 & 3;
  const int lp = ((s >> 1) * H1 + 2 * q + (s & 1)) * 64;
  int aoff[9];
#pragma unroll
  for (int ky = 0; ky < 3; ++ky)
#pragma unroll
    for (int kx = 0; kx < 3; ++kx)
      aoff[ky * 3 + kx] = lp + (ky * H1 + kx) * 64 + ((g ^ ((2 * q + (s & 1) + kx) & 3)) << 4);
  const int pr = wave >> 1;
  const int tt0 = pr < 2 ? 10 * pr : 20 + 8 * (pr - 2), tt1 = tt0 + (pr < 2 ? 10 : 8);
  for (int tt = tt0; tt < tt1; ++tt) {
    const int py = tt / 3, px0 = 4 * (tt - py * 3);
    const char* tb = a1s + (2 * py * H1 + 2 * px0) * 64;
    bf16x8 a[9];
#pragma unroll
    for (int t = 0; t < 9; ++t) a[t] = *reinterpret_cast<const bf16x8*>(tb + aoff[t]);
    f32x4 acc[2];
#pragma unroll
    for (int j = 0; j < 2; ++j) acc[j] = f32x4{b2r[j], b2r[j], b2r[j], b2r[j]};
#pragma unroll
    for (int t = 0; t < 9; ++t)
#pragma unroll
      for (int j = 0; j < 2; ++j)
        acc[j] = __builtin_amdgcn_mfma_f32_16x16x32_bf16(a[t], wb[t][j], acc[j], 0, 0, 0);
    const int pp = py * HP + px0 + g;
#pragma unroll
    for (int j = 0; j < 2; ++j) {
      const int co = nh * 32 + j * 16 + i16;
      const int b0 = fbits(acc[j][0]), b1 = fbits(acc[j][1]), b2 = fbits(acc[j][2]);
      const int mb = max(max(max(b0, b1), b2), fbits(acc[j][3]));
      uint32_t oh = b2 == mb ? 4u : 8u;
      oh = b1 == mb ? 2u : oh;
      oh = b0 == mb ? 1u : oh;
      const bool pos = mb > 0;
      ps[pp * C2 + co] = to_bf16(__builtin_bit_cast(float, max(mb, 0)));
      ms[pp * C2 + co] = (uint8_t)(pos ? 0x80u | oh : 0u);
    }
  }
  PDM_STAMP(3);
  if ((threadIdx.x & 63) == 0 && wave >= 1 && wave <= 6) PDM_STAMP_VAL(9 + wave, PDM_CLOCK());
  __syncthreads();
  PDM_STAMP(4);

  uint4* pout = reinterpret_cast<uint4*>(pool + (int64_t)img * FEAT);
  for (int i = tid; i < FEAT * 2 / 16; i += FWD_THREADS) st_ho<4>(pout + i, reinterpret_cast<const uint4*>(ps)[i]);
  if (TRAIN) {
    uint4* mout = reinterpret_cast<uint4*>(pmask + (int64_t)img * FEAT);
    for (int i = tid; i < FEAT / 16; i += FWD_THREADS) st_ho<4>(mout + i, reinterpret_cast<const uint4*>(ms)[i]);
  }
  if (tid == 64) st_ho<4>(ylab + img, lab);
  PDM_STAMP(5);
}

}

void launch_cnn_fwd(const uint8_t* images, const int32_t* labels, const int32_t* idx,
                    int64_t nrow, const int64_t* ctr, StepRows sr, int B, const float* w1, const float* b1,
                    const __bf16* w2, const float* b2, __bf16* pool, uint8_t* pmask, uint8_t* xg,
                    int32_t* ylab, const FcUpdate* fcc, hipStream_t st) {
  if (fcc != nullptr) {
    cnn_fwd_kernel<true, true><<<B + FCC_WGS, FWD_THREADS, 0, st>>>(
        images, labels, idx, nrow, ctr, sr, w1, b1, w2, b2, pool, pmask, xg, ylab, *fcc, B);
    return;
  }
  const FcUpdate none{};
  if (xg != nullptr)
    cnn_fwd_kernel<true, false><<<B, FWD_THREADS, 0, st>>>(images, labels, idx, nrow, ctr, sr, w1, b1,
                                                           w2, b2, pool, pmask, xg, ylab, none, B);
  else
    cnn_fwd_kernel<false, false><<<B, FWD_THREADS, 0, st>>>(images, labels, idx, nrow, ctr, sr, w1,
                                                            b1, w2, b2, pool, pmask, xg, ylab, none, B);
}

PDM_STAMP_READER(fwd)
```

csrc/kernels/fc1_bwd.hip:

```cpp
#include "cnn_common.h"
#include "optim_common.h"

namespace {

using namespace cnn;

#ifdef PDM_STAMPS
#define FC_STAMP(row, slot)                                                         \
  do {                                                                              \
    if (threadIdx.x == 0 && (row) < 256)                                            \
      pdm_stamps[(row) * 16 + (slot)] = __builtin_amdgcn_s_memtime();              \
  } while (0)
#else
#define FC_STAMP(row, slot) do { } while (0)
#endif
#ifndef PDM_DW_MT
#define PDM_DW_MT 1
#endif
constexpr int DW_MT = PDM_DW_MT;
static_assert(DW_MT == 1 || DW_MT == 2, "dW tile: 64 or 128 hidden rows");
constexpr int DW_FT = FEAT / 64;
constexpr int DW_TILES = DW_FT * (2 / DW_MT);
constexpr int DWC = 128;
constexpr int DX_COLS = 384;
constexpr int DX_TILES = FEAT / DX_COLS;
constexpr int DX_FT = DX_COLS / 64;
constexpr int NXCD = 8;
static_assert(DX_TILES % NXCD == 0 && DW_TILES % NXCD == 0, "XCD-aware tile mapping");
constexpr int HR_BLOCKS = (HEAD_SLAB + 63) / 64;

__device__ __forceinline__ int tile_off(int row, int byte) {
  return row * 128 + (byte ^ ((((row >> 1) & 1) | (((row >> 3) & 1) << 1)) << 5));
}

__global__ __launch_bounds__(256, 2) void fc1_bwd_kernel(
    const bf16* __restrict__ dh, const bf16* __restrict__ dht, int ldt,
    const bf16* __restrict__ pool, const bf16* __restrict__ wf1t, int B, float* __restrict__ gwf1,
    bf16* __restrict__ dpool, const float* __restrict__ head_slab, int head_blocks,
    float* __restrict__ gwf2, float* __restrict__ gbf2, float* __restrict__ gbf1,
    double* __restrict__ metrics, int bid_offset, const FcUpdate fcu) {
  __shared__ __attribute__((aligned(16))) char tile[2 * DWC * 128];
  const int tid = threadIdx.x, lane = tid & 63, wave = tid >> 6;
  const int g = lane >> 4, i16 = lane & 15, q = i16 >> 2, pq = i16 & 3;
  const int nd = (ldt / 32) * DX_TILES;
  const int bid = blockIdx.x + bid_offset;

  if (bid < DW_TILES) {
    const int k0 = (bid % DW_FT) * 64, n0 = (bid / DW_FT) * 64 * DW_MT;
    FC_STAMP(bid, 8);
    f32x4 acc[DW_MT][4];
#pragma unroll
    for (int i = 0; i < DW_MT; ++i)
#pragma unroll
      for (int j = 0; j < 4; ++j) acc[i][j] = f32x4{0.f, 0.f, 0.f, 0.f};
    const int srow = tid >> 3, sch = tid & 7;
    uint4 pv[DWC / 32];
    bf16x8 a[DW_MT][DWC / 32];
    auto load_chunk = [&](int c0) __attribute__((always_inline)) {
#pragma unroll
      for (int j = 0; j < DWC / 32; ++j) {
        const int row = c0 + srow + 32 * j;
        const uint4 v = *reinterpret_cast<const uint4*>(pool + (int64_t)min(row, B - 1) * FEAT +
                                                        k0 + sch * 8);
        pv[j] = row < B ? v : make_uint4(0, 0, 0, 0);
      }
#pragma unroll
      for (int mt = 0; mt < DW_MT; ++mt)
#pragma unroll
        for (int kk = 0; kk < DWC / 32; ++kk)
          a[mt][kk] = *reinterpret_cast<const bf16x8*>(
              dht + ((int64_t)((n0 / 16 + wave * DW_MT + mt) * (ldt / 32) +
                               (min(c0 + 32 * kk, ldt - 32) >> 5)) * 64 + lane) * 8);
    };
    load_chunk(0);
    float fpv[DW_MT][4][4], fmv[DW_MT][4][4];
    double fc_lr = 0.0;
    int64_t fc_t = 0;
    if (fcu.kind >= 0) {
      fc_lr = *fcu.lr;
      fc_t = *fcu.step;
#pragma unroll
      for (int mt = 0; mt < DW_MT; ++mt)
#pragma unroll
        for (int r = 0; r < 4; ++r)
#pragma unroll
          for (int nt = 0; nt < 4; ++nt) {
            const int64_t q = (int64_t)(n0 + wave * 16 * DW_MT + mt * 16 + 4 * g + r) * FEAT + k0 +
                              16 * nt + i16;
            fpv[mt][r][nt] = fcu.p[q];
            fmv[mt][r][nt] = fcu.m[q];
          }
    }
    for (int c0 = 0; c0 < ldt; c0 += DWC) {
      __syncthreads();
#pragma unroll
      for (int j = 0; j < DWC / 32; ++j)
        *reinterpret_cast<uint4*>(tile + tile_off(srow + 32 * j, sch * 16)) = pv[j];
      bf16x8 ac[DW_MT][DWC / 32];
#pragma unroll
      for (int mt = 0; mt < DW_MT; ++mt)
#pragma unroll
        for (int kk = 0; kk < DWC / 32; ++kk) ac[mt][kk] = a[mt][kk];
      __syncthreads();
      FC_STAMP(bid, c0 == 0 ? 9 : 10);
      if (c0 + DWC < ldt) load_chunk(c0 + DWC);
      __builtin_amdgcn_sched_barrier(0);
      const int nk = min(DWC / 32, (ldt - c0) / 32);
#pragma unroll
      for (int kk = 0; kk < DWC / 32; ++kk) {
        if (kk < nk) {
#pragma unroll
          for (int nt = 0; nt < 4; ++nt) {
            const s16x4 lo = lds_tr16(tile + tile_off(32 * kk + 8 * g + q, 32 * nt + 8 * pq));
            const s16x4 hi = lds_tr16(tile + tile_off(32 * kk + 8 * g + 4 + q, 32 * nt + 8 * pq));
            const bf16x8 bv = cat_tr(lo, hi);
#pragma unroll
            for (int mt = 0; mt < DW_MT; ++mt)
              acc[mt][nt] = __builtin_amdgcn_mfma_f32_16x16x32_bf16(ac[mt][kk], bv, acc[mt][nt], 0, 0, 0);
          }
        }
      }
    }
    FC_STAMP(bid, 11);
    if (fcu.kind < 0 || fcu.store_grad) {
#pragma unroll
      for (int mt = 0; mt < DW_MT; ++mt)
#pragma unroll
        for (int r = 0; r < 4; ++r) {
          const int n = n0 + wave * 16 * DW_MT + mt * 16 + 4 * g + r;
#pragma unroll
          for (int nt = 0; nt < 4; ++nt) st_ho<2>(&gwf1[(int64_t)n * FEAT + k0 + 16 * nt + i16], acc[mt][nt][r]);
        }
    }
    if (fcu.kind >= 0) {
      using namespace optim_detail;
      const Hyper h = make_hyper<OPT_SGD>(fcu, fc_lr, fc_t);
      __syncthreads();
      bf16* fr = reinterpret_cast<bf16*>(tile);
      bf16* frt = reinterpret_cast<bf16*>(tile + DWC * 128);
#pragma unroll
      for (int mt = 0; mt < DW_MT; ++mt)
#pragma unroll
        for (int nt = 0; nt < 4; ++nt) {
          bf16 pt[4];
          const int nl0 = wave * 16 * DW_MT + mt * 16 + 4 * g;
#pragma unroll
          for (int r = 0; r < 4; ++r) {
            const int nl = nl0 + r, kl = 16 * nt + i16;
            const int64_t q = (int64_t)(n0 + nl) * FEAT + k0 + kl;
            float m = fmv[mt][r][nt], v = 0.f;
            const float p = update<OPT_SGD>(fpv[mt][r][nt], acc[mt][nt][r], m, v, h, fcu.grad_scale);
            st_ho<2>(&fcu.p[q], p);
            st_ho<2>(&fcu.m[q], m);
            pt[r] = to_bf16(p);
            fr[(((nl >> 4) * 2 + (kl >> 5)) * 64 + ((kl >> 3) & 3) * 16 + (nl & 15)) * 8 + (kl & 7)] = pt[r];
          }
          if (fcu.shadow_t_next != nullptr)
            *reinterpret_cast<bf16x4*>(frt + (((nt * (2 * DW_MT) + (nl0 >> 5)) * 64 +
                                               (((nl0 >> 4) & 1) * 2 + (g >> 1)) * 16 + i16) * 8 +
                                              (g & 1) * 4)) = bf16x4{pt[0], pt[1], pt[2], pt[3]};
        }
      __syncthreads();
#pragma unroll
      for (int u = 0; u < 2 * DW_MT; ++u) {
        const int c = tid + 256 * u, blk = c >> 6;
        st_ho<2>(reinterpret_cast<uint4*>(fcu.shadow + ((int64_t)((n0 / 16 + (blk >> 1)) * (FEAT / 32) +
                                                                   (k0 >> 5) + (blk & 1)) * 64 + (c & 63)) * 8),
                 reinterpret_cast<const uint4*>(fr)[c]);
      }
      if (fcu.shadow_t_next != nullptr) {
#pragma unroll
        for (int u = 0; u < 2 * DW_MT; ++u) {
          const int c = tid + 256 * u, lb = c >> 6;
          const int64_t gb = (int64_t)(k0 / 16 + lb / (2 * DW_MT)) * (HID / 32) + n0 / 32 +
                             lb % (2 * DW_MT);
          st_ho<2>(reinterpret_cast<uint4*>(fcu.shadow_t_next) + gb * 64 + (c & 63),
                   reinterpret_cast<const uint4*>(frt)[c]);
        }
      }
    }
    FC_STAMP(bid, 13);
    return;
  }

  if (bid < DW_TILES + nd) {
    const int t = bid - DW_TILES;
    FC_STAMP(t, 0);
    constexpr int TPX = DX_TILES / NXCD;
    const int xcd = t % NXCD, loc = t / NXCD;
    const int b0 = (loc / TPX) * 32;
    const int f0 = (xcd * TPX + loc % TPX) * DX_COLS + wave * (16 * DX_FT);
    bf16x8 wa[DX_FT][HID / 32], hb[2][HID / 32];
#pragma unroll
    for (int ks = 0; ks < HID / 32; ++ks) {
#pragma unroll
      for (int bt = 0; bt < 2; ++bt)
        hb[bt][ks] = *reinterpret_cast<const bf16x8*>(
            dh + ((int64_t)(((b0 >> 4) + bt) * (HID / 32) + ks) * 64 + lane) * 8);
#pragma unroll
      for (int ft = 0; ft < DX_FT; ++ft)
        wa[ft][ks] = *reinterpret_cast<const bf16x8*>(
            wf1t + ((int64_t)(((f0 >> 4) + ft) * (HID / 32) + ks) * 64 + lane) * 8);
    }
    __builtin_amdgcn_sched_barrier(0);
    FC_STAMP(t, 1);
    f32x4 acc[DX_FT][2];
#pragma unroll
    for (int ft = 0; ft < DX_FT; ++ft)
#pragma unroll
      for (int bt = 0; bt < 2; ++bt) acc[ft][bt] = f32x4{0.f, 0.f, 0.f, 0.f};
#pragma unroll
    for (int ks = 0; ks < HID / 32; ++ks)
#pragma unroll
      for (int ft = 0; ft < DX_FT; ++ft)
#pragma unroll
        for (int bt = 0; bt < 2; ++bt)
          acc[ft][bt] = __builtin_amdgcn_mfma_f32_16x16x32_bf16(hb[bt][ks], wa[ft][ks], acc[ft][bt], 0, 0, 0);
    FC_STAMP(t, 2);
#pragma unroll
    for (int bt = 0; bt < 2; ++bt)
#pragma unroll
      for (int r = 0; r < 4; ++r) {
        const int row = b0 + bt * 16 + 4 * g + r;
        if (row < B) {
#pragma unroll
          for (int ft = 0; ft < DX_FT; ++ft)
            st_ho<2>(&dpool[(int64_t)row * FEAT + f0 + ft * 16 + i16], to_bf16(acc[ft][bt][r]));
        }
      }
    FC_STAMP(t, 3);
    return;
  }

  {
    __shared__ float rs[4][64];
    __shared__ double rd[4][64];
    const int e = (bid - DW_TILES - nd) * 64 + (tid & 63), grp = tid >> 6;
    const int ec = min(e, HEAD_SLAB - 1);
    float s = 0.f;
    double sd = 0.0;
    for (int j0 = grp; j0 < head_blocks; j0 += 4 * 8) {
      float v[8];
#pragma unroll
      for (int u = 0; u < 8; ++u)
        v[u] = head_slab[(int64_t)min(j0 + 4 * u, head_blocks - 1) * HEAD_SLAB + ec];
      __builtin_amdgcn_sched_barrier(0);
#pragma unroll
      for (int u = 0; u < 8; ++u) {
        const float x = (j0 + 4 * u < head_blocks) ? v[u] : 0.f;
        s += x;
        sd += (double)x;
      }
    }
    rs[grp][tid & 63] = s;
    rd[grp][tid & 63] = sd;
    __syncthreads();
    if (tid < 64 && e < HEAD_SLAB) {
      s = ((rs[0][tid] + rs[1][tid]) + rs[2][tid]) + rs[3][tid];
      sd = ((rd[0][tid] + rd[1][tid]) + rd[2][tid]) + rd[3][tid];
      if (e < NCLS * HID) gwf2[e] = s;
      else if (e < NCLS * HID + NCLS) gbf2[e - NCLS * HID] = s;
      else if (e < NCLS * HID + NCLS + HID) gbf1[e - NCLS * HID - NCLS] = s;
      else if (e == HEAD_SLAB - 2) { metrics[0] += sd; metrics[2] += (double)B; }
      else metrics[1] += sd;
    }
  }
}

}

void launch_fc1_bwd(const __bf16* dh, const __bf16* dht, int ldt, const __bf16* pool,
                    const __bf16* wf1t, int B, float* gwf1, __bf16* dpool, const float* head_slab,
                    int head_blocks, float* gwf2, float* gbf2, float* gbf1, double* metrics,
                    const FcUpdate& fcu, hipStream_t st) {
  const int nd = (ldt / 32) * DX_TILES;
  const int nblk = DW_TILES + nd + HR_BLOCKS, off = 0;
  fc1_bwd_kernel<<<nblk, 256, 0, st>>>(dh, dht, ldt, pool, wf1t, B, gwf1, dpool, head_slab,
                                       head_blocks, gwf2, gbf2, gbf1, metrics, off, fcu);
}

PDM_STAMP_READER(fc1_bwd)
```

pytorch_distributed_mnist_amd/runtime/cnn_step.py:

```python
from __future__ import annotations

import os

import torch

from .gpu_step import GpuStepBase

EVAL_CHUNK = 2048


def frag_major(w: torch.Tensor) -> torch.Tensor:
    m, k = w.shape
    t = w.reshape(m // 16, 16, k // 32, 4, 8)
    return t.permute(0, 2, 3, 1, 4).contiguous().reshape(-1)


def a1_swizzled(a1: torch.Tensor) -> torch.Tensor:
    b = a1.shape[0]
    t = a1.reshape(b, 26, 26, 4, 8)
    x = torch.arange(26).view(1, 1, 26, 1)
    src = torch.arange(4).view(1, 1, 1, 4) ^ (x & 3)
    out = torch.gather(t, 3, src.expand(b, 26, 26, 4).unsqueeze(-1).expand(b, 26, 26, 4, 8))
    return out.reshape(-1).contiguous()


def frag_major_t(w: torch.Tensor) -> torch.Tensor:
    return frag_major(w.t())


FC1_BIG_B = 2048


def choose_splitk(B: int, cap: int = 32, target_blocks: int = 256) -> int:
    mtiles = (B + 31) // 32 if B < FC1_BIG_B else (B + 127) // 128
    best = 1
    for s in (1, 2, 4, 8, 16, 32, 48, 96):
        if s <= cap and mtiles * s <= target_blocks:
            best = s
    return best


def choose_ipb(B: int, cus: int = 256) -> int:
    return max(1, -(-B // cus))


BAND_CHOICES = (6, 3, 2)


def choose_bands(B: int, cus: int = 256, forced=None) -> int:
    if forced is not None:
        return int(forced)
    for s in BAND_CHOICES:
        if B * s <= cus:
            return s
    return 1


def conv_blocks(C, B: int, bands_forced=None) -> int:
    bands = choose_bands(B, forced=bands_forced)
    return C.cnn_bwd_nblk(B, choose_ipb(B) if bands == 1 else 1, bands)


class CnnStep(GpuStepBase):
    def __init__(self, prog, use_graphs):
        super().__init__(prog, use_graphs)
        C, dev, B = self.C, self.device, self.bfull
        a = self.arena
        st = self.structure
        bf16 = torch.bfloat16
        self.ldt = -(-B // 32) * 32
        cap = max(B, EVAL_CHUNK)
        self.pool = torch.empty(cap * 9216, dtype=bf16, device=dev)
        self.pmask = torch.empty(cap * 9216, dtype=torch.uint8, device=dev)
        self.xg = torch.empty(B * 784, dtype=torch.uint8, device=dev)
        self.ylab = torch.empty(cap, dtype=torch.int32, device=dev)
        self.splitk_train = choose_splitk(B, cap=st.splitk_cap)
        self.splitk_eval = choose_splitk(min(cap, EVAL_CHUNK))
        part_n = max(self.splitk_train * B, self.splitk_eval * EVAL_CHUNK) * 128
        self.part = torch.empty(part_n, dtype=torch.float32, device=dev)
        self.dh = torch.zeros(self.ldt * 128, dtype=bf16, device=dev)
        self.dht = torch.zeros(self.ldt * 128, dtype=bf16, device=dev)
        self.head_slab = torch.empty(C.cnn_head_nblk(self.ldt) * C.CNN_HEAD_SLAB, dtype=torch.float32,
                                     device=dev)
        self.dpool = torch.empty(B * 9216, dtype=bf16, device=dev)
        self.ipb = choose_ipb(B)
        nband = max(b for b in range(1, B + 1) if self.bands(b) > 1) if \
            any(self.bands(b) > 1 for b in range(1, B + 1)) else 0
        self.a1g = torch.empty(max(nband, 1) * 676 * 32, dtype=bf16, device=dev)
        self.xng = torch.empty(max(nband, 1) * 784, dtype=bf16, device=dev)
        self.conv_nblk = max(conv_blocks(C, b, st.bands) for b in range(1, B + 1))
        self.conv_slab = torch.empty(self.conv_nblk * C.CNN_CONV_SLAB, dtype=torch.float32,
                                     device=dev)
        self.wf1 = torch.empty(128 * 9216, dtype=bf16, device=dev)
        self.wf1t2 = torch.empty(2, 9216 * 128, dtype=bf16, device=dev)
        self.wf1t = self.wf1t2[0]
        self.w2 = torch.empty(64 * 288, dtype=bf16, device=dev)
        self.w2t = torch.empty(288 * 64, dtype=bf16, device=dev)
        p, g = a.param, a.grad
        self.P = {n: p(n) for n in ("conv1.weight", "conv1.bias", "conv2.bias", "fc1.bias",
                                    "fc2.weight", "fc2.bias")}
        self.G = {n: g(n) for n in ("conv1.weight", "conv1.bias", "conv2.weight", "conv2.bias",
                                    "fc1.weight", "fc1.bias", "fc2.weight", "fc2.bias")}
        self.fuse_conv_reduce = not self.reducer.active and st.fuse_conv_reduce
        self.fuse_fc1 = self.fuse_conv_reduce and self.opt.kind == "sgd" and st.fuse_fc1
        self.wt_double = st.fc1_wt_double
        self.keep_grads = st.keep_grads
        self.phase_period = 2 if self._wt_double_on() else 1
        self._fused = {}
        self.xgmi_exchange = st.xgmi_exchange
        self.shard_fc = False
        self._shard_rows = None
        self._side = None
        self._side_ev = None
        self._ema_noticed = False
        self.set_rccl_mode(st.rccl_mode, invalidate=False)
        self.refresh_shadows()
        self._poison_unkept_grads()

    RCCL_MODES = ("carry", "nocarry", "side", "early")

    def bands(self, B: int) -> int:
        return choose_bands(B, forced=self.structure.bands)

    def set_rccl_mode(self, mode: str, invalidate: bool = True) -> None:
        if mode not in self.RCCL_MODES + ("zero",):
            raise ValueError(f"RCCL step mode {mode!r}: choose from {self.RCCL_MODES + ('zero',)}")
        mode = self.rccl_mode_offered(mode)
        shard = mode == "zero"
        if shard:
            mode = "carry"
        self.fc_carry = mode in ("carry", "side")
        self.fc_side = mode == "side"
        self.fc_early = mode == "early"
        if shard and self.reducer.active:
            why = self.shard_unsupported_reason()
            if why is not None:
                raise ValueError(f"RCCL step mode 'zero' (sharded fc1 update): {why}")
            self.set_shard_fc(True)
        if invalidate:
            self.invalidate_graphs()

    def rccl_mode_offered(self, mode: str) -> str:
        if self.ema is None or mode not in ("carry", "side", "zero"):
            return mode
        if self.reducer.active and self.reducer.comm.rank == 0 and not self._ema_noticed:
            self._ema_noticed = True
            print(f"notice: --ema-decay: the RCCL step mode '{mode}' leaves a step's fc1 update "
                  "to a later launch; running 'nocarry'", flush=True)
        return "nocarry"

    def shard_supported(self, reducer=None) -> bool:
        return self.shard_unsupported_reason(reducer) is None

    def shard_world_size(self, reducer=None) -> int:
        red = reducer or self.reducer
        ws = red.comm.world_size
        emu = self.structure.emulate_ws
        return int(emu) if (emu and ws == 1) else ws

    def shard_unsupported_reason(self, reducer=None):
        red = reducer or self.reducer
        ws = self.shard_world_size(red)
        if self.ema is not None:
            return ("the weight average (--ema-decay) takes in every step's whole weights on "
                    "every rank")
        if not red.active:
            return "no gradient reduction at world size 1"
        if not red.can_shard:
            return f"the {red.kind} gradient transport has no reduce-scatter"
        if 128 % ws or (128 // ws) % 16:
            return (f"world size {ws} does not split fc1's 128 rows into shards of a multiple "
                    "of 16 rows")
        return None

    def set_shard_fc(self, on: bool) -> None:
        if bool(on) == self.shard_fc:
            return
        if on:
            if not self.shard_supported():
                raise RuntimeError("fc1 sharding needs an RCCL or gloo data plane and a world "
                                   "size that splits 128 rows into multiples of 16")
            ws, r = self.shard_world_size(), self.reducer.comm.rank
            rows = 128 // ws
            self.reducer.set_shard(0, self.arena.spec.offset("fc1.weight"), rows * 9216)
            self._shard_rows = (r * rows, rows)
            self.shard_fc = True
        else:
            self.sync_master()
            self.reducer.clear_shard()
            self.shard_fc = False
            self._shard_rows = None
        self.invalidate_graphs()

    @torch.no_grad()
    def sync_master(self) -> None:
        if not self.shard_fc:
            return
        off, n = self.arena.spec.offset("fc1.weight"), 128 * 9216
        for buf in (self.arena.params, *self.opt.state_buffers().values()):
            self.reducer.gather(buf[off:off + n])
        self.reducer.wait_gather()

    def _shard_segments(self):
        if getattr(self, "_ssegs", None) is None:
            off1 = self.arena.spec.offset("fc1.weight")
            r0, rows = self._shard_rows
            segs = []
            for sg in self.optimizer_segments():
                if sg[0] == off1:
                    segs.append((off1 + r0 * 9216, rows, 9216,
                                 self.wf1[r0 * 9216:(r0 + rows) * 9216], None, None, False, False,
                                 True))
                else:
                    segs.append(sg)
            tseg = [(off1, 128, 9216, self.wf1, self.wf1t, None, True, True, True)]
            self._ssegs = (segs, tseg)
        return self._ssegs

    @torch.no_grad()
    def refresh_shadows(self) -> None:
        self.sync_master()
        w1 = self.arena.param("fc1.weight").reshape(128, 9216)
        self.wf1.copy_(frag_major(w1.to(torch.bfloat16)))
        wt = frag_major_t(w1.to(torch.bfloat16))
        self.wf1t2[0].copy_(wt)
        self.wf1t2[1].copy_(wt)
        w2 = self.arena.param("conv2.weight").reshape(64, 288)
        self.w2.copy_(frag_major(w2.to(torch.bfloat16)))
        self.w2t.copy_(w2.t().contiguous().reshape(-1).to(torch.bfloat16))

    def optimizer_segments(self):
        spec = self.arena.spec
        segs = []
        for p in spec.params:
            off = spec.offset(p.name)
            if p.name == "fc1.weight":
                segs.append((off, 128, 9216, self.wf1, self.wf1t, None, False, True, True))
            elif p.name == "conv2.weight":
                segs.append((off, 64, 288, self.w2, self.w2t, None, False, False, True))
            else:
                segs.append((off, 1, p.numel, None, None))
        return segs

    def _bucket_segments(self):
        if getattr(self, "_bsegs", None) is None:
            if self._opt_segments is None:
                self._opt_segments = self.optimizer_segments()
            (s0, e0), _ = self.arena.spec.bucket_bounds()
            b0 = [sg for sg in self._opt_segments if s0 <= sg[0] < e0]
            b1 = [sg for sg in self._opt_segments if not (s0 <= sg[0] < e0)]
            self._bsegs = (b0, b1)
        return self._bsegs

    def _fused_segments(self, nblk: int, skip_fc1: bool = False):
        segs = self._fused.get((nblk, skip_fc1))
        if segs is None:
            if self._opt_segments is None:
                self._opt_segments = self.optimizer_segments()
            C = self.C
            col = {"conv2.weight": 0, "conv2.bias": C.CNN_CONV_SLAB_DB2,
                   "conv1.weight": C.CNN_CONV_SLAB_DW1, "conv1.bias": C.CNN_CONV_SLAB_DB1}
            by_off = {self.arena.spec.offset(n): n for n in col}
            slab_segs, plain = [], []
            fc1_off = self.arena.spec.offset("fc1.weight")
            for sg in self._opt_segments:
                name = by_off.get(sg[0])
                if name is None and skip_fc1 and sg[0] == fc1_off:
                    continue
                if name is None and self.fuse_fc1 and sg[0] == fc1_off:
                    if not self.wt_double:
                        plain.append((sg[0], sg[1], sg[2], sg[3], sg[4], None, True, True, True))
                elif name is None:
                    plain.append(sg)
                else:
                    sg = tuple(sg) + (None,) * (9 - len(sg))
                    slab_segs.append(sg[:5] + ((self.conv_slab, nblk, col[name], C.CNN_CONV_SLAB),) +
                                     sg[6:])
            segs = slab_segs + plain
            self._fused[(nblk, skip_fc1)] = segs
        return segs

    def _segments_without_fc1(self):
        if self._opt_segments is None:
            self._opt_segments = self.optimizer_segments()
        off = self.arena.spec.offset("fc1.weight")
        return [sg for sg in self._opt_segments if sg[0] != off]

    def _local_carry(self, B: int) -> bool:
        st = self.structure
        return (not self.reducer.active and self.fuse_fc1 and st.fc1_carry_fwd and
                st.fc1_carry_local and self.bands(B) == 1 and self.ema is None)

    def _fwd_carry_on(self, B: int) -> bool:
        red = self.reducer
        if self.ema is not None:
            return False
        if not red.active:
            return self._local_carry(B)
        if not (self.structure.fc1_carry_fwd and self.opt.kind == "sgd") or self.shard_fc:
            return False
        if self._xchg():
            return True
        return (getattr(red, "kind", None) == "rccl" and getattr(red, "_native", None) is not None
                and not self.fc_carry and not self.fc_early)

    def _fc_carry(self):
        u = self._fc_update()
        return u[:16] + (self.current_wf1t(),)

    def _fc_carry_wait(self):
        red = self.reducer
        if not red.streamed:
            return None
        ch = red.channel_of(self.arena.spec.offset("fc1.weight"))
        return (red.sync, ch, int(red._native.blocks(ch)), float(red.timeout_s))

    def fwd_outputs(self, B: int):
        fb = self.bands(B)
        if fb > 1:
            return None, self.ylab, fb, self.a1g, self.xng
        return self.xg, self.ylab, fb, None, None

    def collective_channels(self):
        return 1 if self._xchg() else None

    def collective_wide(self, B: int) -> bool:
        return self.bands(B) >= 3

    def carries_across_graphs(self, B: int) -> bool:
        return self._fwd_carry_on(B) and self.structure.fc1_carry_graphs

    def _train_seq(self, B: int, n: int, collective: bool = True, cin: bool = False,
                   cout: bool = False) -> None:
        rccl = self.reducer.active and getattr(self.reducer, "kind", None) == "rccl"
        carry = rccl and (self.shard_fc or (self.fc_carry and not self.fc_early))
        fwd = self._fwd_carry_on(B)
        streamed = self.reducer.streamed and collective
        if streamed:
            self.reducer.begin(n, self.collective_channels(), self.collective_wide(B))
        for i in range(n):
            self._train_impl(B, carry_in=carry and i > 0, carry_out=carry and i < n - 1,
                             fwd_in=fwd and (i > 0 or cin), fwd_out=fwd and (i < n - 1 or cout))
            self.launch_ema()
            self.phase = (self.phase + 1) % self.phase_period
        if streamed:
            self.reducer.end()

    def _train_impl(self, B: int, carry_in: bool = False, carry_out: bool = False,
                    fwd_in: bool = False, fwd_out: bool = False) -> None:
        C, P, G = self.C, self.P, self.G
        red = self.reducer
        xs = red.sync if red.streamed else None
        ldt = -(-B // 32) * 32
        S = self.splitk_train
        bands = self.bands(B)
        C.cnn_fwd(self.ep_images.view(-1, 784), self.ep_labels, None, self.ctr[0:1], self.bfull, B,
                  P["conv1.weight"], P["conv1.bias"], self.w2, P["conv2.bias"], self.pool,
                  self.pmask, *self.fwd_outputs(B), spe=self.spe,
                  fc_carry=self._fc_carry() if fwd_in else None,
                  fc_carry_wait=self._fc_carry_wait() if fwd_in else None)
        if carry_in and self.shard_fc:
            self.reducer.wait_gather()
            self.launch_optimizer(self._shard_segments()[1])
        elif carry_in and self.fc_side:
            torch.cuda.current_stream(self.device).wait_event(self._side_ev)
        elif carry_in:
            self.reducer.wait_bucket(0)
            self.launch_optimizer(self._bucket_segments()[0])
        C.fc1_fwd(self.pool, self.wf1, self.part, B, S)
        self.launch_head_train(self.part, S, B, P["fc1.bias"], P["fc2.weight"], P["fc2.bias"],
                               self.ylab, self.dh, self.dht, ldt, self.head_slab,
                               self.metrics.train_view(), self.ctr[0:1], self.opt._step_dev, xs)
        C.fc1_bwd(self.dh, self.dht, ldt, self.pool, self.current_wf1t(), B, G["fc1.weight"], self.dpool,
                  self.head_slab, G["fc2.weight"], G["fc2.bias"], G["fc1.bias"],
                  self.metrics.train_view(),
                  self._fc_update(store_grad=self._local_carry(self.bfull))
                  if self.fuse_fc1 and not fwd_out else None)
        xgmi = getattr(self.reducer, "kind", None) == "xgmi"
        rccl_early = (self.fc_early and not xgmi and red.active and
                      getattr(red, "_native", None) is not None)
        early = xgmi and not red.streamed and self.structure.xgmi_early
        if rccl_early:
            self.reducer.bucket_ready(0)
        if early:
            self.reducer.bucket_ready(0)
        ipb = choose_ipb(B) if bands == 1 else 1
        nblk = C.cnn_bwd_nblk(B, ipb, bands)
        C.cnn_bwd(self.xg, P["conv1.weight"], P["conv1.bias"], self.dpool, self.pmask, self.w2t, B,
                  ipb, self.conv_slab, xs, bands, self.a1g, self.xng)
        if self.fuse_conv_reduce:
            self.launch_optimizer(self._fused_segments(nblk, skip_fc1=fwd_out))
            return
        if self._xchg():
            self.launch_optimizer(self._fused_segments(nblk, skip_fc1=fwd_out), exchange=True)
            return
        C.conv_reduce(self.conv_slab, nblk, G["conv2.weight"], G["conv2.bias"],
                      G["conv1.weight"], G["conv1.bias"])
        if self.shard_fc:
            if not rccl_early:
                self.reducer.bucket_ready(0)
            self.reducer.bucket_ready(1)
            self.reducer.finalize()
            segs, tseg = self._shard_segments()
            self.launch_optimizer(segs)
            self.reducer.gather(self.wf1)
            if not carry_out:
                self.reducer.wait_gather()
                self.launch_optimizer(tseg)
            return
        if xgmi and red.streamed:
            self.launch_optimizer(signal_ch=red.channels_of(1)[0])
            return
        if xgmi:
            if not early:
                self.reducer.bucket_ready(0)
            self.reducer.bucket_ready(1)
            self.reducer.finalize()
            self.launch_optimizer()
            return
        if getattr(self.reducer, "_native", None) is None:
            self.reducer.bucket_ready(0)
            self.reducer.bucket_ready(1)
            self.reducer.finalize()
            self.launch_optimizer()
            return
        if rccl_early:
            self.reducer.bucket_ready(1)
            self.reducer.finalize()
            self.launch_optimizer()
            return
        if not self.fc_carry:
            self.reducer.all_ready()
            self.reducer.finalize()
            self.launch_optimizer(self._segments_without_fc1() if fwd_out else None)
            return
        b0, b1 = self._bucket_segments()
        self.reducer.bucket_ready(1)
        self.reducer.bucket_ready(0)
        if self.fc_side:
            if self._side is None:
                self._side = torch.cuda.Stream(self.device)
                self._side_ev = torch.cuda.Event()
            with torch.cuda.stream(self._side):
                self.reducer.wait_bucket(0)
                self.launch_optimizer(b0)
                self._side_ev.record(self._side)
            self.reducer.wait_bucket(1)
            self.launch_optimizer(b1)
            if not carry_out:
                torch.cuda.current_stream(self.device).wait_event(self._side_ev)
            return
        self.reducer.wait_bucket(1)
        self.launch_optimizer(b1)
        if not carry_out:
            self.reducer.wait_bucket(0)
            self.launch_optimizer(b0)

    def _xchg(self) -> bool:
        red = self.reducer
        return (red.active and getattr(red, "kind", None) == "xgmi" and red.streamed and
                self.xgmi_exchange and red.exchange_ok(1))

    def _fc_update(self, store_grad: bool = False):
        o = self.opt
        g = o.param_groups[0]
        off = self.arena.spec.offset("fc1.weight")
        n = 128 * 9216
        return (self.C.OPT_SGD, self.arena.params[off:off + n], self.reducer.out_grads[off:off + n],
                o.momentum_buffer[off:off + n], None, self.wf1, o._lr_dev, o._step_dev, 0.0, 0.0,
                0.0, float(g["weight_decay"]), float(g["momentum"]), float(g["dampening"]),
                bool(g["nesterov"]), float(self.reducer.grad_scale),
                self.wf1t2[1 - self.phase] if self._wt_double_on() else None,
                self.keep_grads or store_grad)

    def _wt_double_on(self) -> bool:
        return self.fuse_fc1 and self.fuse_conv_reduce and self.wt_double

    def current_wf1t(self) -> torch.Tensor:
        return self.wf1t2[self.phase] if self._wt_double_on() else self.wf1t

    def invalidate_graphs(self) -> None:
        super().invalidate_graphs()
        self._bsegs = None
        self._ssegs = None
        self._fused = {}
        period = 2 if self._wt_double_on() else 1
        if self.phase != self.phase % period:
            self.wf1t2[0].copy_(self.wf1t2[self.phase])
        self.phase_period = period
        self.phase %= period
        self._poison_unkept_grads()

    def _poison_unkept_grads(self) -> None:
        if self.fuse_fc1 and self.fuse_conv_reduce and not self.keep_grads:
            self.G["fc1.weight"].fill_(float("nan"))

    @torch.no_grad()
    def weight_set(self, arena):
        bf16 = torch.bfloat16
        w1 = arena.param("fc1.weight").reshape(128, 9216)
        w2 = arena.param("conv2.weight").reshape(64, 288)
        return ({n: arena.param(n) for n in self.P}, frag_major(w2.to(bf16)),
                frag_major(w1.to(bf16)))

    def evaluate(self, ws=None) -> None:
        C = self.C
        P, w2, wf1 = (self.P, self.w2, self.wf1) if ws is None else ws
        n = self.test_images.shape[0]
        S = self.splitk_eval
        for s in range(0, n, EVAL_CHUNK):
            b = min(EVAL_CHUNK, n - s)
            C.cnn_fwd(self.test_images[s:s + b], self.test_labels[s:s + b], None, None, b, b,
                      P["conv1.weight"], P["conv1.bias"], w2, P["conv2.bias"], self.pool,
                      self.pmask, None, self.ylab)
            C.fc1_fwd(self.pool, wf1, self.part, b, S)
            C.cnn_head(self.part, S, b, P["fc1.bias"], P["fc2.weight"], P["fc2.bias"], self.ylab,
                       False, None, None, 32, None, self.metrics.eval_view(), None, None)

    def predict(self, images_u8, labels=None, ws=None):
        C = self.C
        P, w2, wf1 = (self.P, self.w2, self.wf1) if ws is None else ws
        images, lab, logp, pred, conf = self._predict_io(images_u8, labels)
        n = images.shape[0]
        flab = lab if lab is not None else torch.zeros(n, dtype=torch.int32, device=self.device)
        S = self.splitk_eval
        for s in range(0, n, EVAL_CHUNK):
            b = min(EVAL_CHUNK, n - s)
            C.cnn_fwd(images[s:s + b], flab[s:s + b], None, None, b, b,
                      P["conv1.weight"], P["conv1.bias"], w2, P["conv2.bias"], self.pool,
                      self.pmask, None, self.ylab)
            C.fc1_fwd(self.pool, wf1, self.part, b, S)
            C.cnn_predict_head(self.part, S, b, P["fc1.bias"], P["fc2.weight"], P["fc2.bias"],
                               self.ylab if lab is not None else None, logp[s:s + b],
                               pred[s:s + b], conf)
        return logp, pred, conf
```

pytorch_distributed_mnist_amd/runtime/structure.py:

```python
from __future__ import annotations

from dataclasses import dataclass, replace
from typing import Optional

from .. import knobs

RCCL_MODES = ("carry", "nocarry", "side", "early", "zero")


@dataclass(frozen=True)
class StepStructure:
    rccl_mode: str = "nocarry"
    splitk_cap: int = 32
    fc1_carry_fwd: bool = True
    fc1_carry_graphs: bool = True
    fc1_carry_local: bool = True
    fuse_conv_reduce: bool = True
    fuse_fc1: bool = True
    fc1_wt_double: bool = True
    keep_grads: bool = False
    bands: Optional[int] = None
    xgmi_early: bool = True
    xgmi_exchange: bool = True
    xgmi_outside: bool = True
    fuse_lin_reduce: bool = True
    f32_conv: str = "x3"
    f32_upw: Optional[int] = None
    f32_ipb: Optional[int] = None
    emulate_ws: Optional[int] = None

    def __post_init__(self):
        if self.rccl_mode not in RCCL_MODES:
            raise ValueError(f"RCCL step mode {self.rccl_mode!r}: choose from {RCCL_MODES}")
        if self.f32_conv not in ("x3", "exact"):
            raise ValueError(f"PDM_F32_CONV={self.f32_conv!r}: x3 or exact")

    @classmethod
    def from_env(cls) -> "StepStructure":
        def flag(name, default):
            v = knobs.get(name)
            return default if v is None else v != "0"

        def opt_int(name):
            v = knobs.get(name)
            return None if v is None else int(v)

        d = cls()
        return cls(rccl_mode=knobs.get("PDM_RCCL_MODE", d.rccl_mode),
                   splitk_cap=int(knobs.get("PDM_SPLITK_CAP", str(d.splitk_cap))),
                   fc1_carry_fwd=flag("PDM_FC1_CARRY_FWD", d.fc1_carry_fwd),
                   fc1_carry_graphs=flag("PDM_FC1_CARRY_GRAPHS", d.fc1_carry_graphs),
                   fc1_carry_local=flag("PDM_FC1_CARRY_LOCAL", d.fc1_carry_local),
                   fuse_conv_reduce=flag("PDM_FUSE_CONV_REDUCE", d.fuse_conv_reduce),
                   fuse_fc1=flag("PDM_FUSE_FC1", d.fuse_fc1),
                   fc1_wt_double=flag("PDM_FC1_WT2", d.fc1_wt_double),
                   keep_grads=knobs.get("PDM_KEEP_GRADS", "0") == "1",
                   bands=opt_int("PDM_BANDS"),
                   xgmi_outside=flag("PDM_XGMI_OUTSIDE", d.xgmi_outside),
                   xgmi_exchange=flag("PDM_XGMI_XCHG", d.xgmi_exchange) and
                   knobs.get("PDM_SHARE_DEVICE") != "1",
                   fuse_lin_reduce=flag("PDM_FUSE_LIN_REDUCE", d.fuse_lin_reduce),
                   f32_conv=knobs.get("PDM_F32_CONV", d.f32_conv),
                   f32_upw=opt_int("PDM_F32_UPW"), f32_ipb=opt_int("PDM_F32_IPB"),
                   emulate_ws=opt_int("PDM_EMULATE_WS"))

    def with_(self, **kw) -> "StepStructure":
        return replace(self, **kw)
```

Measured before the change: 4.548 million images/sec.

## Carry fc1 weight-gradient tiles into next step's forward kernel

Moves the fc1 weight-gradient GEMM and fused SGD update out of the fc1 backward kernel and into extra workgroups of the next step's conv forward launch. This lets it overlap with conv work on the single-GPU local path. The pool buffer is double-buffered by phase so the previous step's activations stay readable while the new forward writes. The forward kernel variant uses a higher occupancy bound, and the refactor moves the dW tile code into a shared header. In exchange it adds buffer lifetime coupling across steps and could raise register pressure.

After: 4.553 million images/sec (median of 5 runs). Within noise of the previous version (+0.1%).

```diff
diff --git a/csrc/bind.cpp b/csrc/bind.cpp
--- a/csrc/bind.cpp
+++ b/csrc/bind.cpp
@@ -513,9 +513,32 @@
              at::Tensor w2, at::Tensor b2, at::Tensor pool, at::Tensor pmask,
              c10::optional<at::Tensor> xg, at::Tensor ylab, int64_t bands,
              c10::optional<at::Tensor> a1g, c10::optional<at::Tensor> xng, int64_t spe,
-             c10::optional<py::tuple> fc_carry, c10::optional<py::tuple> fc_carry_wait) {
+             c10::optional<py::tuple> fc_carry, c10::optional<py::tuple> fc_carry_wait,
+             c10::optional<py::tuple> fc_dw_carry) {
   c10::DeviceGuard g(images.device());
   FcUpdate fcc = make_fc_update(fc_carry);
+  FcDwCarry fdw{};
+  if (fc_dw_carry.has_value()) {
+    const py::tuple& d = *fc_dw_carry;
+    TORCH_CHECK(fcc.kind < 0 && !fc_carry_wait.has_value(), "fc_dw_carry replaces fc_carry");
+    TORCH_CHECK(d.size() == 5, "fc_dw_carry: (fc_update, dht, ldt, pool, B)");
+    TORCH_CHECK(bands == 1, "fc_dw_carry: the one-image forward only");
+    fcc = make_fc_update(d[0].cast<py::tuple>());
+    auto dht = d[1].cast<at::Tensor>(), ppool = d[3].cast<at::Tensor>();
+    const int64_t pldt = d[2].cast<int64_t>(), pB = d[4].cast<int64_t>();
+    TORCH_CHECK(pB >= 1 && pldt % 32 == 0 && pldt >= pB, "fc_dw_carry: bad ldt/B");
+    need_min(dht, at::kBFloat16, pldt * CNN_HID, "fc_dw_carry dht");
+    need_min(ppool, at::kBFloat16, pB * CNN_FEAT, "fc_dw_carry pool");
+    const char* r0 = reinterpret_cast<const char*>(ppool.data_ptr());
+    const char* w0 = reinterpret_cast<const char*>(pool.data_ptr());
+    TORCH_CHECK(w0 + B * CNN_FEAT * 2 <= r0 || r0 + pB * CNN_FEAT * 2 <= w0,
+                "fc_dw_carry: the previous step's pool overlaps the pool this launch writes");
+    fdw.dht = ptr<__bf16>(dht);
+    fdw.pool = ptr<__bf16>(ppool);
+    fdw.ldt = (int)pldt;
+    fdw.B = (int)pB;
+  }
+  const FcDwCarry* pfdw = fdw.dht != nullptr ? &fdw : nullptr;
   if (fc_carry_wait.has_value()) {
     const py::tuple& w = *fc_carry_wait;
     TORCH_CHECK(fcc.kind >= 0 && w.size() == 4, "fc_carry_wait: (sync, channel, mult, timeout_s) "
@@ -593,7 +616,7 @@
     launch_cnn_fwd(images.data_ptr<uint8_t>(), labels.data_ptr<int32_t>(), pidx, nrow, pctr,
                    step_rows(bfull, pidx ? 0 : spe, nrow), (int)B, w1.data_ptr<float>(), b1.data_ptr<float>(), ptr<__bf16>(w2),
                    b2.data_ptr<float>(), ptr<__bf16>(pool), pmask.data_ptr<uint8_t>(), pxg,
-                   ylab.data_ptr<int32_t>(), pfcc, cur_stream(images));
+                   ylab.data_ptr<int32_t>(), pfcc, pfdw, cur_stream(images));
   }
 }
 
@@ -858,9 +881,10 @@
 void fc1_bwd(at::Tensor dh, at::Tensor dht, int64_t ldt, at::Tensor pool, at::Tensor wf1t,
              int64_t B, at::Tensor gwf1, at::Tensor dpool, at::Tensor head_slab, at::Tensor gwf2,
              at::Tensor gbf2, at::Tensor gbf1, at::Tensor metrics,
-             c10::optional<py::tuple> fc_update) {
+             c10::optional<py::tuple> fc_update, bool dw_carried) {
   c10::DeviceGuard g(dh.device());
   TORCH_CHECK(B >= 1 && ldt % 32 == 0 && ldt >= B, "bad ldt/B");
+  TORCH_CHECK(!(dw_carried && fc_update.has_value()), "dw_carried: no fc_update in this launch");
   need_min(dh, at::kBFloat16, ldt * CNN_HID, "dh");
   need_min(dht, at::kBFloat16, ldt * CNN_HID, "dht");
   need_min(pool, at::kBFloat16, B * CNN_FEAT, "pool");
@@ -886,7 +910,7 @@
   launch_fc1_bwd(ptr<__bf16>(dh), ptr<__bf16>(dht), (int)ldt, ptr<__bf16>(pool), ptr<__bf16>(wf1t),
                  (int)B, gwf1.data_ptr<float>(), ptr<__bf16>(dpool), head_slab.data_ptr<float>(),
                  (int)hb, gwf2.data_ptr<float>(), gbf2.data_ptr<float>(), gbf1.data_ptr<float>(),
-                 metrics.data_ptr<double>(), fcu, cur_stream(dh));
+                 metrics.data_ptr<double>(), fcu, dw_carried, cur_stream(dh));
 }
 
 static int64_t conv_blocks(int64_t B, int64_t ipb, int64_t bands) {
@@ -1135,7 +1159,8 @@
         py::arg("bfull"), py::arg("B"), py::arg("w1"), py::arg("b1"), py::arg("w2"), py::arg("b2"),
         py::arg("pool"), py::arg("pmask"), py::arg("xg"), py::arg("ylab"), py::arg("bands") = 1,
         py::arg("a1g") = py::none(), py::arg("xng") = py::none(), py::arg("spe") = 0,
-        py::arg("fc_carry") = py::none(), py::arg("fc_carry_wait") = py::none());
+        py::arg("fc_carry") = py::none(), py::arg("fc_carry_wait") = py::none(),
+        py::arg("fc_dw_carry") = py::none());
   m.def("fc1_fwd", &fc1_fwd);
   m.attr("FC1_BIG_B") = FC1_BIG_B;
   m.def("cnn_head", &cnn_head, py::arg("part"), py::arg("splitk"), py::arg("B"), py::arg("bf1"),
@@ -1165,7 +1190,7 @@
   m.def("fc1_bwd", &fc1_bwd, py::arg("dh"), py::arg("dht"), py::arg("ldt"), py::arg("pool"),
         py::arg("wf1t"), py::arg("B"), py::arg("gwf1"), py::arg("dpool"), py::arg("head_slab"),
         py::arg("gwf2"), py::arg("gbf2"), py::arg("gbf1"), py::arg("metrics"),
-        py::arg("fc_update") = py::none());
+        py::arg("fc_update") = py::none(), py::arg("dw_carried") = false);
   m.def("cnn_bwd", &cnn_bwd, py::arg("xg"), py::arg("w1"), py::arg("b1"), py::arg("dpool"),
         py::arg("pmask"), py::arg("w2t"), py::arg("B"), py::arg("ipb"), py::arg("slab"),
         py::arg("xg_sync") = py::none(), py::arg("bands") = 1, py::arg("a1g") = py::none(),
diff --git a/csrc/kernels.h b/csrc/kernels.h
--- a/csrc/kernels.h
+++ b/csrc/kernels.h
@@ -155,10 +155,16 @@
 constexpr int CNN_CONV_SLAB_DW1 = 18496;
 constexpr int CNN_CONV_SLAB_DB1 = 18784;
 
+struct FcDwCarry {
+  const __bf16* dht;
+  const __bf16* pool;
+  int ldt, B;
+};
+
 void launch_cnn_fwd(const uint8_t* images, const int32_t* labels, const int32_t* idx,
                     int64_t nrow, const int64_t* ctr, StepRows sr, int B, const float* w1, const float* b1,
                     const __bf16* w2, const float* b2, __bf16* pool, uint8_t* pmask, uint8_t* xg,
-                    int32_t* ylab, const FcUpdate* fcc, hipStream_t st);
+                    int32_t* ylab, const FcUpdate* fcc, const FcDwCarry* fdw, hipStream_t st);
 void launch_cnn_fwd_band(const uint8_t* images, const int32_t* labels, const int32_t* idx,
                          int64_t nrow, const int64_t* ctr, StepRows sr, int B, int bands,
                          const float* w1, const float* b1, const __bf16* w2, const float* b2,
@@ -187,7 +193,7 @@
 void launch_fc1_bwd(const __bf16* dh, const __bf16* dht, int ldt, const __bf16* pool,
                     const __bf16* wf1t, int B, float* gwf1, __bf16* dpool, const float* head_slab,
                     int head_blocks, float* gwf2, float* gbf2, float* gbf1, double* metrics,
-                    const FcUpdate& fcu, hipStream_t st);
+                    const FcUpdate& fcu, bool dw_carried, hipStream_t st);
 void launch_cnn_bwd(const uint8_t* xg, const float* w1, const float* b1, const __bf16* dpool,
                     const uint8_t* pmask, const __bf16* w2t, int B, int imgs_per_block, float* slab,
                     unsigned* xg_sync, hipStream_t st);
diff --git a/csrc/kernels/cnn_fwd.hip b/csrc/kernels/cnn_fwd.hip
--- a/csrc/kernels/cnn_fwd.hip
+++ b/csrc/kernels/cnn_fwd.hip
@@ -1,5 +1,6 @@
 #include "cnn_common.h"
 #include "fc_carry.h"
+#include "fc1_dw.h"
 
 namespace {
 
@@ -15,18 +16,30 @@
 constexpr int F_TOTAL = F_W + 1536;
 static_assert(2 * F_TOTAL <= 163840 && F_A1 % 128 == 0, "cnn_fwd LDS carve");
 
-template <bool TRAIN, bool CARRY>
-__global__ __launch_bounds__(FWD_THREADS, 2) void cnn_fwd_kernel(
+enum { CARRY_NONE = 0, CARRY_UPDATE = 1, CARRY_DW = 2 };
+constexpr int DW_WGS = DW_TILES / 2;
+template <bool TRAIN, int CARRY>
+__device__ __forceinline__ void cnn_fwd_body(
     const uint8_t* __restrict__ images, const int32_t* __restrict__ labels,
     const int32_t* __restrict__ idx, int64_t nrow, const int64_t* __restrict__ ctr, const StepRows sr,
     const float* __restrict__ w1, const float* __restrict__ b1, const bf16* __restrict__ w2,
     const float* __restrict__ b2, bf16* __restrict__ pool, uint8_t* __restrict__ pmask,
-    uint8_t* __restrict__ xg, int32_t* __restrict__ ylab, const FcUpdate fcc, int nconv) {
+    uint8_t* __restrict__ xg, int32_t* __restrict__ ylab, const FcUpdate fcc, const FcDwCarry fdw,
+    int nconv) {
   __shared__ __attribute__((aligned(16))) char smem[F_TOTAL];
   static_assert(F_TOTAL >= FCC_LDS + 4, "carried fc1 update tiles fit the forward's LDS");
-  if constexpr (CARRY) {
+  static_assert(F_TOTAL >= 2 * DW_LDS, "two carried dW tiles fit the forward's LDS");
+  if constexpr (CARRY == CARRY_UPDATE) {
     if ((int)blockIdx.x >= nconv) {
       fc_carry_role(fcc, blockIdx.x - nconv, gridDim.x - nconv, smem);
+      return;
+    }
+  }
+  if constexpr (CARRY == CARRY_DW) {
+    if ((int)blockIdx.x >= nconv) {
+      const int half = threadIdx.x >> 8;
+      fc1_dw_tile((int)blockIdx.x - nconv + half * DW_WGS, threadIdx.x & 255, smem + half * DW_LDS,
+                  fdw.dht, fdw.ldt, fdw.pool, fdw.B, const_cast<float*>(fcc.g), fcc);
       return;
     }
   }
@@ -196,24 +209,48 @@
   PDM_STAMP(5);
 }
 
+#define CNN_FWD_PARAMS                                                                         \
+  const uint8_t *__restrict__ images, const int32_t *__restrict__ labels,                      \
+      const int32_t *__restrict__ idx, int64_t nrow, const int64_t *__restrict__ ctr,          \
+      const StepRows sr, const float *__restrict__ w1, const float *__restrict__ b1,           \
+      const bf16 *__restrict__ w2, const float *__restrict__ b2, bf16 *__restrict__ pool,      \
+      uint8_t *__restrict__ pmask, uint8_t *__restrict__ xg, int32_t *__restrict__ ylab,       \
+      const FcUpdate fcc, const FcDwCarry fdw, int nconv
+#define CNN_FWD_ARGS \
+  images, labels, idx, nrow, ctr, sr, w1, b1, w2, b2, pool, pmask, xg, ylab, fcc, fdw, nconv
+
+template <bool TRAIN, int CARRY>
+__global__ __launch_bounds__(FWD_THREADS, 2) void cnn_fwd_kernel(CNN_FWD_PARAMS) {
+  cnn_fwd_body<TRAIN, CARRY>(CNN_FWD_ARGS);
+}
+__global__ __launch_bounds__(FWD_THREADS, 4) void cnn_fwd_kernel_dw(CNN_FWD_PARAMS) {
+  cnn_fwd_body<true, CARRY_DW>(CNN_FWD_ARGS);
+}
+
 }
 
 void launch_cnn_fwd(const uint8_t* images, const int32_t* labels, const int32_t* idx,
                     int64_t nrow, const int64_t* ctr, StepRows sr, int B, const float* w1, const float* b1,
                     const __bf16* w2, const float* b2, __bf16* pool, uint8_t* pmask, uint8_t* xg,
-                    int32_t* ylab, const FcUpdate* fcc, hipStream_t st) {
+                    int32_t* ylab, const FcUpdate* fcc, const FcDwCarry* fdw, hipStream_t st) {
+  const FcDwCarry nodw{};
+  if (fcc != nullptr && fdw != nullptr) {
+    cnn_fwd_kernel_dw<<<B + DW_WGS, FWD_THREADS, 0, st>>>(
+        images, labels, idx, nrow, ctr, sr, w1, b1, w2, b2, pool, pmask, xg, ylab, *fcc, *fdw, B);
+    return;
+  }
   if (fcc != nullptr) {
-    cnn_fwd_kernel<true, true><<<B + FCC_WGS, FWD_THREADS, 0, st>>>(
-        images, labels, idx, nrow, ctr, sr, w1, b1, w2, b2, pool, pmask, xg, ylab, *fcc, B);
+    cnn_fwd_kernel<true, CARRY_UPDATE><<<B + FCC_WGS, FWD_THREADS, 0, st>>>(
+        images, labels, idx, nrow, ctr, sr, w1, b1, w2, b2, pool, pmask, xg, ylab, *fcc, nodw, B);
     return;
   }
   const FcUpdate none{};
   if (xg != nullptr)
-    cnn_fwd_kernel<true, false><<<B, FWD_THREADS, 0, st>>>(images, labels, idx, nrow, ctr, sr, w1, b1,
-                                                           w2, b2, pool, pmask, xg, ylab, none, B);
+    cnn_fwd_kernel<true, CARRY_NONE><<<B, FWD_THREADS, 0, st>>>(
+        images, labels, idx, nrow, ctr, sr, w1, b1, w2, b2, pool, pmask, xg, ylab, none, nodw, B);
   else
-    cnn_fwd_kernel<false, false><<<B, FWD_THREADS, 0, st>>>(images, labels, idx, nrow, ctr, sr, w1,
-                                                            b1, w2, b2, pool, pmask, xg, ylab, none, B);
+    cnn_fwd_kernel<false, CARRY_NONE><<<B, FWD_THREADS, 0, st>>>(
+        images, labels, idx, nrow, ctr, sr, w1, b1, w2, b2, pool, pmask, xg, ylab, none, nodw, B);
 }
 
 PDM_STAMP_READER(fwd)
diff --git a/csrc/kernels/fc1_bwd.hip b/csrc/kernels/fc1_bwd.hip
--- a/csrc/kernels/fc1_bwd.hip
+++ b/csrc/kernels/fc1_bwd.hip
@@ -1,9 +1,4 @@
 #include "cnn_common.h"
-#include "optim_common.h"
-
-namespace {
-
-using namespace cnn;
 
 #ifdef PDM_STAMPS
 #define FC_STAMP(row, slot)                                                         \
@@ -14,14 +9,13 @@
 #else
 #define FC_STAMP(row, slot) do { } while (0)
 #endif
-#ifndef PDM_DW_MT
-#define PDM_DW_MT 1
-#endif
-constexpr int DW_MT = PDM_DW_MT;
-static_assert(DW_MT == 1 || DW_MT == 2, "dW tile: 64 or 128 hidden rows");
-constexpr int DW_FT = FEAT / 64;
-constexpr int DW_TILES = DW_FT * (2 / DW_MT);
-constexpr int DWC = 128;
+#define FC1_DW_STAMP(row, slot) FC_STAMP(row, slot)
+#include "fc1_dw.h"
+
+namespace {
+
+using namespace cnn;
+
 constexpr int DX_COLS = 384;
 constexpr int DX_TILES = FEAT / DX_COLS;
 constexpr int DX_FT = DX_COLS / 64;
@@ -29,157 +23,20 @@
 static_assert(DX_TILES % NXCD == 0 && DW_TILES % NXCD == 0, "XCD-aware tile mapping");
 constexpr int HR_BLOCKS = (HEAD_SLAB + 63) / 64;
 
-__device__ __forceinline__ int tile_off(int row, int byte) {
-  return row * 128 + (byte ^ ((((row >> 1) & 1) | (((row >> 3) & 1) << 1)) << 5));
-}
-
 __global__ __launch_bounds__(256, 2) void fc1_bwd_kernel(
     const bf16* __restrict__ dh, const bf16* __restrict__ dht, int ldt,
     const bf16* __restrict__ pool, const bf16* __restrict__ wf1t, int B, float* __restrict__ gwf1,
     bf16* __restrict__ dpool, const float* __restrict__ head_slab, int head_blocks,
     float* __restrict__ gwf2, float* __restrict__ gbf2, float* __restrict__ gbf1,
     double* __restrict__ metrics, int bid_offset, const FcUpdate fcu) {
-  __shared__ __attribute__((aligned(16))) char tile[2 * DWC * 128];
+  __shared__ __attribute__((aligned(16))) char tile[DW_LDS];
   const int tid = threadIdx.x, lane = tid & 63, wave = tid >> 6;
   const int g = lane >> 4, i16 = lane & 15, q = i16 >> 2, pq = i16 & 3;
   const int nd = (ldt / 32) * DX_TILES;
   const int bid = blockIdx.x + bid_offset;
 
   if (bid < DW_TILES) {
-    const int k0 = (bid % DW_FT) * 64, n0 = (bid / DW_FT) * 64 * DW_MT;
-    FC_STAMP(bid, 8);
-    f32x4 acc[DW_MT][4];
-#pragma unroll
-    for (int i = 0; i < DW_MT; ++i)
-#pragma unroll
-      for (int j = 0; j < 4; ++j) acc[i][j] = f32x4{0.f, 0.f, 0.f, 0.f};
-    const int srow = tid >> 3, sch = tid & 7;
-    uint4 pv[DWC / 32];
-    bf16x8 a[DW_MT][DWC / 32];
-    auto load_chunk = [&](int c0) __attribute__((always_inline)) {
-#pragma unroll
-      for (int j = 0; j < DWC / 32; ++j) {
-        const int row = c0 + srow + 32 * j;
-        const uint4 v = *reinterpret_cast<const uint4*>(pool + (int64_t)min(row, B - 1) * FEAT +
-                                                        k0 + sch * 8);
-        pv[j] = row < B ? v : make_uint4(0, 0, 0, 0);
-      }
-#pragma unroll
-      for (int mt = 0; mt < DW_MT; ++mt)
-#pragma unroll
-        for (int kk = 0; kk < DWC / 32; ++kk)
-          a[mt][kk] = *reinterpret_cast<const bf16x8*>(
-              dht + ((int64_t)((n0 / 16 + wave * DW_MT + mt) * (ldt / 32) +
-                               (min(c0 + 32 * kk, ldt - 32) >> 5)) * 64 + lane) * 8);
-    };
-    load_chunk(0);
-    float fpv[DW_MT][4][4], fmv[DW_MT][4][4];
-    double fc_lr = 0.0;
-    int64_t fc_t = 0;
-    if (fcu.kind >= 0) {
-      fc_lr = *fcu.lr;
-      fc_t = *fcu.step;
-#pragma unroll
-      for (int mt = 0; mt < DW_MT; ++mt)
-#pragma unroll
-        for (int r = 0; r < 4; ++r)
-#pragma unroll
-          for (int nt = 0; nt < 4; ++nt) {
-            const int64_t q = (int64_t)(n0 + wave * 16 * DW_MT + mt * 16 + 4 * g + r) * FEAT + k0 +
-                              16 * nt + i16;
-            fpv[mt][r][nt] = fcu.p[q];
-            fmv[mt][r][nt] = fcu.m[q];
-          }
-    }
-    for (int c0 = 0; c0 < ldt; c0 += DWC) {
-      __syncthreads();
-#pragma unroll
-      for (int j = 0; j < DWC / 32; ++j)
-        *reinterpret_cast<uint4*>(tile + tile_off(srow + 32 * j, sch * 16)) = pv[j];
-      bf16x8 ac[DW_MT][DWC / 32];
-#pragma unroll
-      for (int mt = 0; mt < DW_MT; ++mt)
-#pragma unroll
-        for (int kk = 0; kk < DWC / 32; ++kk) ac[mt][kk] = a[mt][kk];
-      __syncthreads();
-      FC_STAMP(bid, c0 == 0 ? 9 : 10);
-      if (c0 + DWC < ldt) load_chunk(c0 + DWC);
-      __builtin_amdgcn_sched_barrier(0);
-      const int nk = min(DWC / 32, (ldt - c0) / 32);
-#pragma unroll
-      for (int kk = 0; kk < DWC / 32; ++kk) {
-        if (kk < nk) {
-#pragma unroll
-          for (int nt = 0; nt < 4; ++nt) {
-            const s16x4 lo = lds_tr16(tile + tile_off(32 * kk + 8 * g + q, 32 * nt + 8 * pq));
-            const s16x4 hi = lds_tr16(tile + tile_off(32 * kk + 8 * g + 4 + q, 32 * nt + 8 * pq));
-            const bf16x8 bv = cat_tr(lo, hi);
-#pragma unroll
-            for (int mt = 0; mt < DW_MT; ++mt)
-              acc[mt][nt] = __builtin_amdgcn_mfma_f32_16x16x32_bf16(ac[mt][kk], bv, acc[mt][nt], 0, 0, 0);
-          }
-        }
-      }
-    }
-    FC_STAMP(bid, 11);
-    if (fcu.kind < 0 || fcu.store_grad) {
-#pragma unroll
-      for (int mt = 0; mt < DW_MT; ++mt)
-#pragma unroll
-        for (int r = 0; r < 4; ++r) {
-          const int n = n0 + wave * 16 * DW_MT + mt * 16 + 4 * g + r;
-#pragma unroll
-          for (int nt = 0; nt < 4; ++nt) st_ho<2>(&gwf1[(int64_t)n * FEAT + k0 + 16 * nt + i16], acc[mt][nt][r]);
-        }
-    }
-    if (fcu.kind >= 0) {
-      using namespace optim_detail;
-      const Hyper h = make_hyper<OPT_SGD>(fcu, fc_lr, fc_t);
-      __syncthreads();
-      bf16* fr = reinterpret_cast<bf16*>(tile);
-      bf16* frt = reinterpret_cast<bf16*>(tile + DWC * 128);
-#pragma unroll
-      for (int mt = 0; mt < DW_MT; ++mt)
-#pragma unroll
-        for (int nt = 0; nt < 4; ++nt) {
-          bf16 pt[4];
-          const int nl0 = wave * 16 * DW_MT + mt * 16 + 4 * g;
-#pragma unroll
-          for (int r = 0; r < 4; ++r) {
-            const int nl = nl0 + r, kl = 16 * nt + i16;
-            const int64_t q = (int64_t)(n0 + nl) * FEAT + k0 + kl;
-            float m = fmv[mt][r][nt], v = 0.f;
-            const float p = update<OPT_SGD>(fpv[mt][r][nt], acc[mt][nt][r], m, v, h, fcu.grad_scale);
-            st_ho<2>(&fcu.p[q], p);
-            st_ho<2>(&fcu.m[q], m);
-            pt[r] = to_bf16(p);
-            fr[(((nl >> 4) * 2 + (kl >> 5)) * 64 + ((kl >> 3) & 3) * 16 + (nl & 15)) * 8 + (kl & 7)] = pt[r];
-          }
-          if (fcu.shadow_t_next != nullptr)
-            *reinterpret_cast<bf16x4*>(frt + (((nt * (2 * DW_MT) + (nl0 >> 5)) * 64 +
-                                               (((nl0 >> 4) & 1) * 2 + (g >> 1)) * 16 + i16) * 8 +
-                                              (g & 1) * 4)) = bf16x4{pt[0], pt[1], pt[2], pt[3]};
-        }
-      __syncthreads();
-#pragma unroll
-      for (int u = 0; u < 2 * DW_MT; ++u) {
-        const int c = tid + 256 * u, blk = c >> 6;
-        st_ho<2>(reinterpret_cast<uint4*>(fcu.shadow + ((int64_t)((n0 / 16 + (blk >> 1)) * (FEAT / 32) +
-                                                                   (k0 >> 5) + (blk & 1)) * 64 + (c & 63)) * 8),
-                 reinterpret_cast<const uint4*>(fr)[c]);
-      }
-      if (fcu.shadow_t_next != nullptr) {
-#pragma unroll
-        for (int u = 0; u < 2 * DW_MT; ++u) {
-          const int c = tid + 256 * u, lb = c >> 6;
-          const int64_t gb = (int64_t)(k0 / 16 + lb / (2 * DW_MT)) * (HID / 32) + n0 / 32 +
-                             lb % (2 * DW_MT);
-          st_ho<2>(reinterpret_cast<uint4*>(fcu.shadow_t_next) + gb * 64 + (c & 63),
-                   reinterpret_cast<const uint4*>(frt)[c]);
-        }
-      }
-    }
-    FC_STAMP(bid, 13);
+    fc1_dw_tile(bid, tid, tile, dht, ldt, pool, B, gwf1, fcu);
     return;
   }
 
@@ -272,9 +129,10 @@
 void launch_fc1_bwd(const __bf16* dh, const __bf16* dht, int ldt, const __bf16* pool,
                     const __bf16* wf1t, int B, float* gwf1, __bf16* dpool, const float* head_slab,
                     int head_blocks, float* gwf2, float* gbf2, float* gbf1, double* metrics,
-                    const FcUpdate& fcu, hipStream_t st) {
+                    const FcUpdate& fcu, bool dw_carried, hipStream_t st) {
   const int nd = (ldt / 32) * DX_TILES;
-  const int nblk = DW_TILES + nd + HR_BLOCKS, off = 0;
+  const int off = dw_carried ? DW_TILES : 0;
+  const int nblk = DW_TILES - off + nd + HR_BLOCKS;
   fc1_bwd_kernel<<<nblk, 256, 0, st>>>(dh, dht, ldt, pool, wf1t, B, gwf1, dpool, head_slab,
                                        head_blocks, gwf2, gbf2, gbf1, metrics, off, fcu);
 }
diff --git a/csrc/kernels/fc1_dw.h b/csrc/kernels/fc1_dw.h
--- /dev/null
+++ b/csrc/kernels/fc1_dw.h
@@ -0,0 +1,167 @@
+#pragma once
+#include "cnn_common.h"
+#include "optim_common.h"
+
+#ifndef FC1_DW_STAMP
+#define FC1_DW_STAMP(row, slot) do { } while (0)
+#endif
+
+namespace cnn {
+
+#ifndef PDM_DW_MT
+#define PDM_DW_MT 1
+#endif
+constexpr int DW_MT = PDM_DW_MT;
+static_assert(DW_MT == 1 || DW_MT == 2, "dW tile: 64 or 128 hidden rows");
+constexpr int DW_FT = FEAT / 64;
+constexpr int DW_TILES = DW_FT * (2 / DW_MT);
+constexpr int DWC = 128;
+constexpr int DW_LDS = 2 * DWC * 128;
+
+__device__ __forceinline__ int dw_tile_off(int row, int byte) {
+  return row * 128 + (byte ^ ((((row >> 1) & 1) | (((row >> 3) & 1) << 1)) << 5));
+}
+
+__device__ __forceinline__ void fc1_dw_tile(int bid, int tid, char* tile,
+                                            const bf16* __restrict__ dht, int ldt,
+                                            const bf16* __restrict__ pool, int B,
+                                            float* __restrict__ gwf1, const FcUpdate& fcu) {
+  const int lane = tid & 63, wave = tid >> 6;
+  const int g = lane >> 4, i16 = lane & 15, q = i16 >> 2, pq = i16 & 3;
+  const int k0 = (bid % DW_FT) * 64, n0 = (bid / DW_FT) * 64 * DW_MT;
+  FC1_DW_STAMP(bid, 8);
+  f32x4 acc[DW_MT][4];
+#pragma unroll
+  for (int i = 0; i < DW_MT; ++i)
+#pragma unroll
+    for (int j = 0; j < 4; ++j) acc[i][j] = f32x4{0.f, 0.f, 0.f, 0.f};
+  const int srow = tid >> 3, sch = tid & 7;
+  uint4 pv[DWC / 32];
+  bf16x8 a[DW_MT][DWC / 32];
+  auto load_chunk = [&](int c0) __attribute__((always_inline)) {
+#pragma unroll
+    for (int j = 0; j < DWC / 32; ++j) {
+      const int row = c0 + srow + 32 * j;
+      const uint4 v = *reinterpret_cast<const uint4*>(pool + (int64_t)min(row, B - 1) * FEAT +
+                                                      k0 + sch * 8);
+      pv[j] = row < B ? v : make_uint4(0, 0, 0, 0);
+    }
+#pragma unroll
+    for (int mt = 0; mt < DW_MT; ++mt)
+#pragma unroll
+      for (int kk = 0; kk < DWC / 32; ++kk)
+        a[mt][kk] = *reinterpret_cast<const bf16x8*>(
+            dht + ((int64_t)((n0 / 16 + wave * DW_MT + mt) * (ldt / 32) +
+                             (min(c0 + 32 * kk, ldt - 32) >> 5)) * 64 + lane) * 8);
+  };
+  load_chunk(0);
+  float fpv[DW_MT][4][4], fmv[DW_MT][4][4];
+  double fc_lr = 0.0;
+  int64_t fc_t = 0;
+  if (fcu.kind >= 0) {
+    fc_lr = *fcu.lr;
+    fc_t = *fcu.step;
+#pragma unroll
+    for (int mt = 0; mt < DW_MT; ++mt)
+#pragma unroll
+      for (int r = 0; r < 4; ++r)
+#pragma unroll
+        for (int nt = 0; nt < 4; ++nt) {
+          const int64_t e = (int64_t)(n0 + wave * 16 * DW_MT + mt * 16 + 4 * g + r) * FEAT + k0 +
+                            16 * nt + i16;
+          fpv[mt][r][nt] = fcu.p[e];
+          fmv[mt][r][nt] = fcu.m[e];
+        }
+  }
+  for (int c0 = 0; c0 < ldt; c0 += DWC) {
+    __syncthreads();
+#pragma unroll
+    for (int j = 0; j < DWC / 32; ++j)
+      *reinterpret_cast<uint4*>(tile + dw_tile_off(srow + 32 * j, sch * 16)) = pv[j];
+    bf16x8 ac[DW_MT][DWC / 32];
+#pragma unroll
+    for (int mt = 0; mt < DW_MT; ++mt)
+#pragma unroll
+      for (int kk = 0; kk < DWC / 32; ++kk) ac[mt][kk] = a[mt][kk];
+    __syncthreads();
+    FC1_DW_STAMP(bid, c0 == 0 ? 9 : 10);
+    if (c0 + DWC < ldt) load_chunk(c0 + DWC);
+    __builtin_amdgcn_sched_barrier(0);
+    const int nk = min(DWC / 32, (ldt - c0) / 32);
+#pragma unroll
+    for (int kk = 0; kk < DWC / 32; ++kk) {
+      if (kk < nk) {
+#pragma unroll
+        for (int nt = 0; nt < 4; ++nt) {
+          const s16x4 lo = lds_tr16(tile + dw_tile_off(32 * kk + 8 * g + q, 32 * nt + 8 * pq));
+          const s16x4 hi = lds_tr16(tile + dw_tile_off(32 * kk + 8 * g + 4 + q, 32 * nt + 8 * pq));
+          const bf16x8 bv = cat_tr(lo, hi);
+#pragma unroll
+          for (int mt = 0; mt < DW_MT; ++mt)
+            acc[mt][nt] = __builtin_amdgcn_mfma_f32_16x16x32_bf16(ac[mt][kk], bv, acc[mt][nt], 0, 0, 0);
+        }
+      }
+    }
+  }
+  FC1_DW_STAMP(bid, 11);
+  if (fcu.kind < 0 || fcu.store_grad) {
+#pragma unroll
+    for (int mt = 0; mt < DW_MT; ++mt)
+#pragma unroll
+      for (int r = 0; r < 4; ++r) {
+        const int n = n0 + wave * 16 * DW_MT + mt * 16 + 4 * g + r;
+#pragma unroll
+        for (int nt = 0; nt < 4; ++nt) st_ho<2>(&gwf1[(int64_t)n * FEAT + k0 + 16 * nt + i16], acc[mt][nt][r]);
+      }
+  }
+  if (fcu.kind >= 0) {
+    using namespace optim_detail;
+    const Hyper h = make_hyper<OPT_SGD>(fcu, fc_lr, fc_t);
+    __syncthreads();
+    bf16* fr = reinterpret_cast<bf16*>(tile);
+    bf16* frt = reinterpret_cast<bf16*>(tile + DWC * 128);
+#pragma unroll
+    for (int mt = 0; mt < DW_MT; ++mt)
+#pragma unroll
+      for (int nt = 0; nt < 4; ++nt) {
+        bf16 pt[4];
+        const int nl0 = wave * 16 * DW_MT + mt * 16 + 4 * g;
+#pragma unroll
+        for (int r = 0; r < 4; ++r) {
+          const int nl = nl0 + r, kl = 16 * nt + i16;
+          const int64_t e = (int64_t)(n0 + nl) * FEAT + k0 + kl;
+          float m = fmv[mt][r][nt], v = 0.f;
+          const float p = update<OPT_SGD>(fpv[mt][r][nt], acc[mt][nt][r], m, v, h, fcu.grad_scale);
+          st_ho<2>(&fcu.p[e], p);
+          st_ho<2>(&fcu.m[e], m);
+          pt[r] = to_bf16(p);
+          fr[(((nl >> 4) * 2 + (kl >> 5)) * 64 + ((kl >> 3) & 3) * 16 + (nl & 15)) * 8 + (kl & 7)] = pt[r];
+        }
+        if (fcu.shadow_t_next != nullptr)
+          *reinterpret_cast<bf16x4*>(frt + (((nt * (2 * DW_MT) + (nl0 >> 5)) * 64 +
+                                             (((nl0 >> 4) & 1) * 2 + (g >> 1)) * 16 + i16) * 8 +
+                                            (g & 1) * 4)) = bf16x4{pt[0], pt[1], pt[2], pt[3]};
+      }
+    __syncthreads();
+#pragma unroll
+    for (int u = 0; u < 2 * DW_MT; ++u) {
+      const int c = tid + 256 * u, blk = c >> 6;
+      st_ho<2>(reinterpret_cast<uint4*>(fcu.shadow + ((int64_t)((n0 / 16 + (blk >> 1)) * (FEAT / 32) +
+                                                                 (k0 >> 5) + (blk & 1)) * 64 + (c & 63)) * 8),
+               reinterpret_cast<const uint4*>(fr)[c]);
+    }
+    if (fcu.shadow_t_next != nullptr) {
+#pragma unroll
+      for (int u = 0; u < 2 * DW_MT; ++u) {
+        const int c = tid + 256 * u, lb = c >> 6;
+        const int64_t gb = (int64_t)(k0 / 16 + lb / (2 * DW_MT)) * (HID / 32) + n0 / 32 +
+                           lb % (2 * DW_MT);
+        st_ho<2>(reinterpret_cast<uint4*>(fcu.shadow_t_next) + gb * 64 + (c & 63),
+                 reinterpret_cast<const uint4*>(frt)[c]);
+      }
+    }
+  }
+  FC1_DW_STAMP(bid, 13);
+}
+
+}
diff --git a/pytorch_distributed_mnist_amd/runtime/cnn_step.py b/pytorch_distributed_mnist_amd/runtime/cnn_step.py
--- a/pytorch_distributed_mnist_amd/runtime/cnn_step.py
+++ b/pytorch_distributed_mnist_amd/runtime/cnn_step.py
@@ -71,6 +71,7 @@
         self.ldt = -(-B // 32) * 32
         cap = max(B, EVAL_CHUNK)
         self.pool = torch.empty(cap * 9216, dtype=bf16, device=dev)
+        self._pool_b = None
         self.pmask = torch.empty(cap * 9216, dtype=torch.uint8, device=dev)
         self.xg = torch.empty(B * 784, dtype=torch.uint8, device=dev)
         self.ylab = torch.empty(cap, dtype=torch.int32, device=dev)
@@ -116,6 +117,7 @@
         self.set_rccl_mode(st.rccl_mode, invalidate=False)
         self.refresh_shadows()
         self._poison_unkept_grads()
+        self._alloc_pool_b()
 
     RCCL_MODES = ("carry", "nocarry", "side", "early")
 
@@ -287,9 +289,27 @@
         return [sg for sg in self._opt_segments if sg[0] != off]
 
     def _local_carry(self, B: int) -> bool:
-        st = self.structure
-        return (not self.reducer.active and self.fuse_fc1 and st.fc1_carry_fwd and
-                st.fc1_carry_local and self.bands(B) == 1 and self.ema is None)
+        return self.fuse_fc1 and self.structure.local_carry(**self._carry_facts(B))
+
+    def _carry_facts(self, B: int) -> dict:
+        return dict(reducing=self.reducer.active, opt_kind=self.opt.kind, ema=self.ema is not None,
+                    bands=self.bands(B))
+
+    def _dw_carry(self, B: int) -> bool:
+        return (self._local_carry(B) and self._wt_double_on() and
+                self.structure.dw_carry(**self._carry_facts(B)))
+
+    def _alloc_pool_b(self) -> None:
+        if self._pool_b is None and self._dw_carry(self.bfull):
+            self._pool_b = torch.empty(self.bfull * 9216, dtype=torch.bfloat16, device=self.device)
+
+    def _step_pool(self, B: int, prev: bool = False) -> torch.Tensor:
+        odd = self._dw_carry(B) and (self.phase == 1) != prev
+        return self._pool_b if odd else self.pool
+
+    def _fc_dw_carry(self, B: int, ldt: int):
+        u = self._fc_update(store_grad=True)
+        return (u[:16] + (self.current_wf1t(), u[17]), self.dht, ldt, self._step_pool(B, prev=True), B)
 
     def _fwd_carry_on(self, B: int) -> bool:
         red = self.reducer
@@ -354,11 +374,14 @@
         ldt = -(-B // 32) * 32
         S = self.splitk_train
         bands = self.bands(B)
+        dwc = self._dw_carry(B)
+        pool = self._step_pool(B)
         C.cnn_fwd(self.ep_images.view(-1, 784), self.ep_labels, None, self.ctr[0:1], self.bfull, B,
-                  P["conv1.weight"], P["conv1.bias"], self.w2, P["conv2.bias"], self.pool,
+                  P["conv1.weight"], P["conv1.bias"], self.w2, P["conv2.bias"], pool,
                   self.pmask, *self.fwd_outputs(B), spe=self.spe,
-                  fc_carry=self._fc_carry() if fwd_in else None,
-                  fc_carry_wait=self._fc_carry_wait() if fwd_in else None)
+                  fc_carry=self._fc_carry() if fwd_in and not dwc else None,
+                  fc_carry_wait=self._fc_carry_wait() if fwd_in and not dwc else None,
+                  fc_dw_carry=self._fc_dw_carry(B, ldt) if fwd_in and dwc else None)
         if carry_in and self.shard_fc:
             self.reducer.wait_gather()
             self.launch_optimizer(self._shard_segments()[1])
@@ -367,15 +390,16 @@
         elif carry_in:
             self.reducer.wait_bucket(0)
             self.launch_optimizer(self._bucket_segments()[0])
-        C.fc1_fwd(self.pool, self.wf1, self.part, B, S)
+        C.fc1_fwd(pool, self.wf1, self.part, B, S)
         self.launch_head_train(self.part, S, B, P["fc1.bias"], P["fc2.weight"], P["fc2.bias"],
                                self.ylab, self.dh, self.dht, ldt, self.head_slab,
                                self.metrics.train_view(), self.ctr[0:1], self.opt._step_dev, xs)
-        C.fc1_bwd(self.dh, self.dht, ldt, self.pool, self.current_wf1t(), B, G["fc1.weight"], self.dpool,
+        C.fc1_bwd(self.dh, self.dht, ldt, pool, self.current_wf1t(), B, G["fc1.weight"], self.dpool,
                   self.head_slab, G["fc2.weight"], G["fc2.bias"], G["fc1.bias"],
                   self.metrics.train_view(),
                   self._fc_update(store_grad=self._local_carry(self.bfull))
-                  if self.fuse_fc1 and not fwd_out else None)
+                  if self.fuse_fc1 and not fwd_out else None,
+                  dw_carried=fwd_out and dwc)
         xgmi = getattr(self.reducer, "kind", None) == "xgmi"
         rccl_early = (self.fc_early and not xgmi and red.active and
                       getattr(red, "_native", None) is not None)
@@ -490,6 +514,7 @@
         self.phase_period = period
         self.phase %= period
         self._poison_unkept_grads()
+        self._alloc_pool_b()
 
     def _poison_unkept_grads(self) -> None:
         if self.fuse_fc1 and self.fuse_conv_reduce and not self.keep_grads:
diff --git a/pytorch_distributed_mnist_amd/runtime/structure.py b/pytorch_distributed_mnist_amd/runtime/structure.py
--- a/pytorch_distributed_mnist_amd/runtime/structure.py
+++ b/pytorch_distributed_mnist_amd/runtime/structure.py
@@ -15,6 +15,7 @@
     fc1_carry_fwd: bool = True
     fc1_carry_graphs: bool = True
     fc1_carry_local: bool = True
+    fc1_dw_carry: bool = True
     fuse_conv_reduce: bool = True
     fuse_fc1: bool = True
     fc1_wt_double: bool = True
@@ -64,5 +65,13 @@
                    f32_upw=opt_int("PDM_F32_UPW"), f32_ipb=opt_int("PDM_F32_IPB"),
                    emulate_ws=opt_int("PDM_EMULATE_WS"))
 
+    def local_carry(self, *, reducing: bool, opt_kind: str, ema: bool, bands: int) -> bool:
+        return (not reducing and opt_kind == "sgd" and self.fuse_conv_reduce and self.fuse_fc1 and
+                self.fc1_carry_fwd and self.fc1_carry_local and bands == 1 and not ema)
+
+    def dw_carry(self, *, reducing: bool, opt_kind: str, ema: bool, bands: int) -> bool:
+        return (self.fc1_dw_carry and self.fc1_wt_double and
+                self.local_carry(reducing=reducing, opt_kind=opt_kind, ema=ema, bands=bands))
+
     def with_(self, **kw) -> "StepStructure":
         return replace(self, **kw)
```
